# SandroMartens/DBGSOM

Measured on AMD Instinct MI355X. Metric: samples/sec/epoch (BMU+update), higher is better.
Workload: dtype f64; 1 GPU; Synthetic N=1e6 d=784 fp32, M=1024 (32x32); samples_total=1000000, samples_per_gpu=1000000, features=784, prototypes=1024, x_storage=f32, map=frozen (same prototypes every step), bmu_algorithm=filtered, via=HipBackend -> dbgsom_ctx_epoch (one C-ABI call per step)

## Files before the change

dbgsom_amd/_native.py:

```python
from __future__ import annotations

import ctypes
import os
import subprocess

_HERE = os.path.dirname(os.path.abspath(__file__))
CSRC = os.path.join(_HERE, "csrc")
LIB_PATH = os.environ.get("DBGSOM_LIB") or os.path.join(CSRC, "libdbgsom_hip.so")
HEADER = os.path.join(os.path.dirname(_HERE), "include", "dbgsom_hip.h")

F32, F64, BF16 = 0, 1, 2
ALG_AUTO, ALG_EXACT, ALG_FILTERED, ALG_FILTERED_HINT = 0, 1, 2, 3
ALGORITHMS = {"auto": ALG_AUTO, "exact": ALG_EXACT, "filtered": ALG_FILTERED,
              "filtered_hint": ALG_FILTERED_HINT}
EPOCH_FROZEN = 1
ABI_VERSION = 4
ALLREDUCE_FN = ctypes.CFUNCTYPE(ctypes.c_int, ctypes.c_void_p, ctypes.c_void_p, ctypes.c_int64,
                                ctypes.c_void_p)
COLLECTIVE_FN = ctypes.CFUNCTYPE(ctypes.c_int, ctypes.c_void_p, ctypes.c_int, ctypes.c_void_p, ctypes.c_int64,
                                 ctypes.c_void_p)
COLL_ALLREDUCE, COLL_REDUCE_SCATTER, COLL_ALLGATHER = 0, 1, 2
CENTRES_COMPACT, CENTRES_ALIGNED = 0, 1
LAYOUTS = {"compact": CENTRES_COMPACT, "aligned": CENTRES_ALIGNED}
MAX_PROTOTYPES = 16000
SC_COUNTS = ("samples", "iterations", "max_iterations", "drops", "degenerate", "early_stops", "aa_retries",
             "overflow", "max_active", "multi_drops", "g_rows")

_i64, _vp, _ci, _dbl, _sz = (ctypes.c_int64, ctypes.c_void_p, ctypes.c_int, ctypes.c_double,
                             ctypes.c_size_t)

SIGNATURES = {
    "dbgsom_abi_version": (_ci, []),
    "dbgsom_last_error": (ctypes.c_char_p, []),
    "dbgsom_device_count": (_ci, [ctypes.POINTER(_ci)]),
    "dbgsom_row_sqnorms": (_ci, [_vp, _ci, _i64, _i64, _i64, _vp, _vp]),
    "dbgsom_bmu": (_ci, [_vp, _ci, _i64, _i64, _i64, _vp, _vp, _i64, _vp, _ci, _ci, _vp, _vp, _vp]),
    "dbgsom_exp_similarity": (_ci, [_vp, _i64, _dbl, _vp, _vp]),
    "dbgsom_accumulate_workspace_bytes": (_sz, [_i64, _i64, _i64]),
    "dbgsom_accumulate": (_ci, [_vp, _ci, _i64, _i64, _i64, _vp, _vp, _vp, _i64, _vp, _vp, _vp,
                                _sz, _vp]),
    "dbgsom_smooth_workspace_bytes": (_sz, [_i64, _i64]),
    "dbgsom_smooth": (_ci, [_vp, _i64, _i64, _vp, _dbl, _ci, _vp, _vp, _vp, _vp, _sz, _vp]),
    "dbgsom_filter_planes_bytes": (_sz, [_i64, _i64]),
    "dbgsom_filter_prepare": (_ci, [_vp, _ci, _i64, _i64, _i64, _vp, _sz, _vp]),
    "dbgsom_bmu_filtered_workspace_bytes": (_sz, [_i64, _i64, _i64]),
    "dbgsom_bmu_filtered": (_ci, [_vp, _ci, _i64, _i64, _i64, _vp, _vp, _vp, _i64, _vp, _vp, _vp,
                                  _ci, _ci, _ci, _vp, _vp, _vp, _sz, _vp]),
    "dbgsom_bmu_filtered_counts": (_ci, [_vp, _i64, _i64, _i64, _vp, _i64, _vp]),
    "dbgsom_bmu_filtered_counts_async": (_ci, [_vp, _i64, _i64, _i64, _vp, _i64, _vp]),
    "dbgsom_bmu_filtered_refine_counts": (_ci, [_vp, _i64, _i64, _i64, _vp, _vp]),
    "dbgsom_bmu_filtered_gaps": (_ci, [_vp, _i64, _i64, _i64, _vp, _vp]),
    "dbgsom_bmu_filtered_anchored": (_ci, [_vp, _ci, _i64, _i64, _i64, _vp, _vp, _vp, _i64, _vp, _vp, _ci, _vp, _vp,
                                           _ci, _ci, _ci, _vp, _vp, _vp, _sz, _vp]),
    "dbgsom_bmu_filtered_anchor_seeds": (_ci, [_vp, _i64, _i64, _i64, _ci, _vp, _vp, _vp]),
    "dbgsom_filter_timing": (_ci, [_ci]),
    "dbgsom_bmu_filtered_stage_ms": (_ci, [_vp]),
    "dbgsom_sum_workspace_bytes": (_sz, []),
    "dbgsom_sum_f64": (_ci, [_vp, _i64, _vp, _vp, _sz, _vp]),
    "dbgsom_column_sums": (_ci, [_vp, _ci, _i64, _i64, _i64, _vp, _vp, _vp]),
    "dbgsom_topographic_count": (_ci, [_vp, _i64, _vp, _i64, _vp, _vp]),
    "dbgsom_density_terms": (_ci, [_vp, _i64, _dbl, _vp, _vp]),
    "dbgsom_class_histogram": (_ci, [_vp, _vp, _i64, _i64, _i64, _vp, _vp]),
    "dbgsom_ctx_create": (_ci, [_ci, ctypes.POINTER(_vp)]),
    "dbgsom_ctx_destroy": (_ci, [_vp]),
    "dbgsom_ctx_set_option": (_ci, [_vp, ctypes.c_char_p, _i64]),
    "dbgsom_ctx_get_option": (_ci, [_vp, ctypes.c_char_p, ctypes.POINTER(_i64)]),
    "dbgsom_ctx_stream": (_ci, [_vp, ctypes.POINTER(_vp)]),
    "dbgsom_ctx_load": (_ci, [_vp, _vp, _ci, _i64, _i64, _ci]),
    "dbgsom_ctx_load_device": (_ci, [_vp, _vp, _ci, _i64, _i64, _i64]),
    "dbgsom_ctx_read_samples": (_ci, [_vp, _vp, _i64, _vp]),
    "dbgsom_ctx_set_labels": (_ci, [_vp, _vp, _i64]),
    "dbgsom_ctx_set_sample_weight": (_ci, [_vp, _vp, _i64]),
    "dbgsom_ctx_weight_total": (_ci, [_vp, _vp]),
    "dbgsom_ctx_weighted_column_sums": (_ci, [_vp, _vp, _vp]),
    "dbgsom_ctx_class_histogram_weighted": (_ci, [_vp, _vp, _i64, _i64, _vp]),
    "dbgsom_accumulate_weighted_workspace_bytes": (_sz, [_i64, _i64, _i64]),
    "dbgsom_accumulate_weighted": (_ci, [_vp, _ci, _i64, _i64, _i64, _vp, _vp, _vp, _vp, _i64, _vp, _vp, _vp,
                                         _sz, _vp]),
    "dbgsom_weighted_sum_f64": (_ci, [_vp, _vp, _i64, _vp, _vp, _sz, _vp]),
    "dbgsom_topographic_weight": (_ci, [_vp, _vp, _i64, _vp, _i64, _vp, _vp, _sz, _vp]),
    "dbgsom_class_histogram_weighted": (_ci, [_vp, _vp, _vp, _vp, _i64, _i64, _i64, _vp, _vp]),
    "dbgsom_weighted_column_sums_workspace_bytes": (_sz, [_i64]),
    "dbgsom_weighted_column_sums": (_ci, [_vp, _ci, _i64, _i64, _i64, _vp, _vp, _vp, _vp, _sz, _vp]),
    "dbgsom_ctx_set_topology": (_ci, [_vp, _vp, _i64]),
    "dbgsom_ctx_set_allreduce": (_ci, [_vp, _vp, _vp]),
    "dbgsom_ctx_set_collectives": (_ci, [_vp, _vp, _vp, _ci, _ci]),
    "dbgsom_rccl_unique_id": (_ci, [_vp]),
    "dbgsom_rccl_comm_init": (_ci, [_vp, _ci, _ci, ctypes.POINTER(_vp)]),
    "dbgsom_rccl_comm_destroy": (_ci, [_vp]),
    "dbgsom_ctx_set_rccl": (_ci, [_vp, _vp]),
    "dbgsom_ctx_allreduce_host": (_ci, [_vp, _vp, _i64]),
    "dbgsom_ctx_set_weights": (_ci, [_vp, _vp, _i64]),
    "dbgsom_ctx_get_weights": (_ci, [_vp, _ci, _vp, _i64]),
    "dbgsom_ctx_read_weight_rows": (_ci, [_vp, _ci, _vp, _i64, _vp]),
    "dbgsom_ctx_write_weight_rows": (_ci, [_vp, _i64, _i64, _vp]),
    "dbgsom_ctx_bmu": (_ci, [_vp, _vp, _i64, _ci, _ci, _vp, _vp]),
    "dbgsom_ctx_bmu_query": (_ci, [_vp, _vp, _ci, _i64, _i64, _vp, _i64, _ci, _ci, _vp, _vp]),
    "dbgsom_ctx_bmu_query_device": (_ci, [_vp, _vp, _ci, _i64, _i64, _i64, _vp, _i64, _ci, _ci, _vp, _vp]),
    "dbgsom_ctx_sparse_code_device": (_ci, [_vp, _vp, _ci, _i64, _i64, _i64, _vp, _i64, _ci, _vp, _i64, _vp, _vp,
                                            _vp]),
    "dbgsom_ctx_topographic_function_device": (_ci, [_vp, _vp, _ci, _i64, _i64, _i64, _vp, _i64, _ci, _vp, _i64, _vp,
                                                     _vp, _vp]),
    "dbgsom_sparse_code_workspace_bytes": (_sz, [_i64, _i64, _i64, _ci]),
    "dbgsom_sparse_code": (_ci, [_vp, _ci, _i64, _i64, _i64, _vp, _i64, _i64, _ci, _ci, _vp, _i64, _vp, _vp, _vp,
                                 _vp, _sz, _vp]),
    "dbgsom_sparse_code_timing": (_ci, [_ci]),
    "dbgsom_sparse_code_stage_ms": (_ci, [_vp]),
    "dbgsom_csr_check": (_ci, [_vp, _vp, _i64, _i64, _i64]),
    "dbgsom_csr_row_sqnorms": (_ci, [_vp, _vp, _ci, _i64, _vp, _vp]),
    "dbgsom_csr_wt_ld": (_i64, [_i64]),
    "dbgsom_csr_transpose_weights": (_ci, [_vp, _i64, _i64, _i64, _vp, _i64, _vp]),
    "dbgsom_bmu_csr": (_ci, [_vp, _vp, _vp, _ci, _i64, _vp, _vp, _i64, _i64, _vp, _ci, _ci, _vp, _vp, _vp]),
    "dbgsom_csr_densify": (_ci, [_vp, _vp, _vp, _ci, _i64, _i64, _i64, _vp, _vp]),
    "dbgsom_accumulate_csr_workspace_bytes": (_sz, [_i64, _i64, _i64]),
    "dbgsom_accumulate_csr": (_ci, [_vp, _vp, _vp, _ci, _i64, _i64, _vp, _vp, _vp, _vp, _i64, _vp, _vp, _vp, _sz,
                                    _vp]),
    "dbgsom_ctx_load_csr": (_ci, [_vp, _vp, _vp, _vp, _ci, _i64, _i64, _i64]),
    "dbgsom_ctx_bmu_query_csr": (_ci, [_vp, _vp, _vp, _vp, _ci, _i64, _i64, _i64, _vp, _i64, _ci, _ci, _vp, _vp]),
    "dbgsom_ctx_sparse_code": (_ci, [_vp, _vp, _ci, _i64, _i64, _vp, _i64, _ci, _vp, _i64, _vp, _vp, _vp]),
    "dbgsom_bmu_masked_workspace_bytes": (_sz, [_ci, _i64, _i64, _i64]),
    "dbgsom_bmu_masked": (_ci, [_vp, _ci, _i64, _i64, _i64, _vp, _i64, _i64, _ci, _vp, _vp, _vp, _sz, _vp]),
    "dbgsom_fill_missing": (_ci, [_vp, _ci, _i64, _i64, _i64, _vp, _i64, _i64, _vp, _i64, _vp]),
    "dbgsom_ctx_bmu_query_masked": (_ci, [_vp, _vp, _ci, _i64, _i64, _vp, _i64, _ci, _vp, _vp, _vp]),
    "dbgsom_accumulate_masked_workspace_bytes": (_sz, [_i64, _i64, _i64]),
    "dbgsom_accumulate_masked": (_ci, [_vp, _ci, _i64, _i64, _i64, _vp, _vp, _vp, _i64, _vp, _vp, _vp, _sz, _vp]),
    "dbgsom_smooth_masked_workspace_bytes": (_sz, [_i64, _i64]),
    "dbgsom_smooth_masked": (_ci, [_vp, _i64, _i64, _vp, _dbl, _vp, _vp, _vp, _vp, _sz, _vp]),
    "dbgsom_ctx_bmu_masked": (_ci, [_vp, _vp, _i64, _ci, _vp, _vp]),
    "dbgsom_ctx_epoch_masked": (_ci, [_vp, _vp, _i64, _dbl, _dbl, _vp, _vp, _vp, _vp, _vp, _vp]),
    "dbgsom_topofn_workspace_bytes": (_sz, [_i64, _ci]),
    "dbgsom_topofn": (_ci, [_vp, _i64, _vp, _i64, _i64, _vp, _vp, _vp, _vp, _sz, _vp]),
    "dbgsom_topofn_timing": (_ci, [_ci]),
    "dbgsom_topofn_stage_ms": (_ci, [_vp]),
    "dbgsom_ctx_topographic_function": (_ci, [_vp, _vp, _ci, _i64, _i64, _vp, _i64, _ci, _vp, _i64, _vp, _vp,
                                              _vp]),
    "dbgsom_ctx_exp_similarity": (_ci, [_vp, _vp, _i64, _dbl, _vp]),
    "dbgsom_ctx_epoch": (_ci, [_vp, _vp, _i64, _ci, _dbl, _dbl, _ci, _ci, _vp, _vp, _vp, _vp, _vp,
                               _vp]),
    "dbgsom_ctx_update": (_ci, [_vp, _vp, _i64, _vp, _vp, _vp, _dbl, _ci, _vp, _vp, _vp, _vp]),
    "dbgsom_ctx_set_hint": (_ci, [_vp, _vp, _i64]),
    "dbgsom_ctx_read_sums": (_ci, [_vp, _vp, _i64]),
    "dbgsom_ctx_column_sums": (_ci, [_vp, _vp, _vp]),
    "dbgsom_ctx_quantization_error": (_ci, [_vp, _vp, _i64, _ci, _vp]),
    "dbgsom_ctx_topographic_count": (_ci, [_vp, _vp, _i64, _ci, _vp, _vp]),
    "dbgsom_ctx_node_statistics": (_ci, [_vp, _vp, _i64, _ci, _dbl, _vp, _vp]),
    "dbgsom_ctx_class_histogram": (_ci, [_vp, _vp, _i64, _i64, _vp]),
    "dbgsom_ctx_partition": (_ci, [_vp, _vp, _i64, _ci, _vp, _vp]),
    "dbgsom_ctx_subset_create": (_ci, [_vp, _i64, ctypes.POINTER(_vp)]),
    "dbgsom_ctx_epoch_info": (_ci, [_vp, _vp]),
    "dbgsom_ctx_arm_ms": (_ci, [_vp, _vp]),
    "dbgsom_ctx_filter_counts": (_ci, [_vp, _vp, _i64]),
    "dbgsom_ctx_read_anchors": (_ci, [_vp, ctypes.POINTER(_i64), _vp, _vp, _vp, _vp]),
    "dbgsom_ctx_refine_counts": (_ci, [_vp, _vp]),
    "dbgsom_ctx_phase_ms": (_ci, [_vp, _vp]),
}

_lib = None
_hip_rt = None


class DbgsomNativeError(RuntimeError):

    def __init__(self, fn, code, msg):
        super().__init__(f"{fn} failed ({code}): {msg}")
        self.code = code


def build(verbose: bool = False) -> str:
    out = None if verbose else subprocess.DEVNULL
    subprocess.check_call(["make", "-C", CSRC, "-j4", "libdbgsom_hip.so"], stdout=out)
    return LIB_PATH


def _load_hip_runtime():
    candidates = []
    try:
        import importlib.util

        spec = importlib.util.find_spec("torch")
        if spec and spec.origin:
            candidates.append(os.path.join(os.path.dirname(spec.origin), "lib", "libamdhip64.so"))
    except (ImportError, ValueError):
        pass
    rocm = os.environ.get("ROCM_PATH", "/opt/rocm")
    candidates += [os.path.join(rocm, "lib", "libamdhip64.so"), "libamdhip64.so"]
    errors = []
    for path in candidates:
        if os.path.isabs(path) and not os.path.exists(path):
            continue
        try:
            rt = ctypes.CDLL(path, mode=ctypes.RTLD_GLOBAL)
        except OSError as e:
            errors.append(f"{path}: {e}")
            continue
        rccl = os.path.join(os.path.dirname(path), "librccl.so") if os.path.isabs(path) else ""
        if rccl and os.path.exists(rccl):
            os.environ.setdefault("DBGSOM_RCCL_LIB", rccl)
        return rt
    raise RuntimeError("no HIP runtime (libamdhip64.so) could be loaded: " + "; ".join(errors))


def load():
    global _lib, _hip_rt
    if _lib is not None:
        return _lib
    if not os.path.exists(LIB_PATH):
        raise RuntimeError(
            f"{LIB_PATH} is missing: the HIP extension is not built. Run "
            "`python -c 'import __graft_entry__ as g; g.build()'` (or `make -C dbgsom_amd/csrc`). "
            "dbgsom_amd has no CPU fallback.")
    _hip_rt = _load_hip_runtime()
    lib = ctypes.CDLL(LIB_PATH)
    for name, (res, args) in SIGNATURES.items():
        fn = getattr(lib, name)
        fn.restype = res
        fn.argtypes = args
    if lib.dbgsom_abi_version() != ABI_VERSION:
        raise RuntimeError(f"ABI version mismatch: library {lib.dbgsom_abi_version()}, "
                           f"binding {ABI_VERSION} (rebuild: make -C dbgsom_amd/csrc)")
    _lib = lib
    return lib


def check(fn_name: str, rc: int) -> None:
    if rc != 0:
        msg = load().dbgsom_last_error()
        err = DbgsomNativeError(fn_name, rc, msg.decode(errors="replace") if msg else "")
        if rc == -1:
            raise ValueError(str(err))
        raise err


def call(fn_name: str, *args):
    check(fn_name, getattr(load(), fn_name)(*args))
# ... 7 lines not shown
```

dbgsom_amd/backend.py:

```python
from __future__ import annotations

import ctypes
import os
from dataclasses import dataclass
from typing import Optional

import numpy as np

from . import _native


@dataclass
class EpochResult:
    new_weights: np.ndarray
    change_total: float
    errors: np.ndarray
    activations: np.ndarray
    winners: Optional[np.ndarray] = None
    distances: Optional[np.ndarray] = None
    new_weights_dev: object = None
    class_hist: Optional[np.ndarray] = None


def shard_bounds(n: int, rank: int, world: int):
# ... 253 lines not shown
_RCCL_COMMS = {}


class HipBackend(HotPathBackend):

    name = "hip"

    FILTER_MIN_PROTOTYPES = 129
    FILTER_MAX_FEATURES = 43690
    FILTER_MAX_MEAN_CANDIDATES = 320
    FILTER_MIN_QUERY_ROWS = 32768
    SWEEP_COST = {1: 0.35, 2: 1.0, 3: 1.96}
    LIST_COST = 12.5
    PRUNE_PASS_COST = 60.0

    def __init__(self, device: Optional[int] = None, algorithm: str = "auto", _ctx=None):
        self._lib = _native.load()
        if algorithm not in _native.ALGORITHMS:
            raise ValueError("algorithm must be 'auto', 'exact', 'filtered' or 'filtered_hint'")
        self._init_args = (device, algorithm)
        n_dev = _native.device_count()
        if n_dev < 1:
            raise RuntimeError(
                "dbgsom_amd.HipBackend needs a visible AMD GPU (MI355X / gfx950); found "
                f"hipGetDeviceCount()={n_dev}. There is no CPU fallback in the product path.")
        if device is None:
            device = int(os.environ.get("LOCAL_RANK", "0")) % n_dev
        self.device_index = int(device)
        self._ctx = ctypes.c_void_p()
        if _ctx is not None:
            self._ctx = _ctx
        else:
            _native.call("dbgsom_ctx_create", self.device_index, ctypes.byref(self._ctx))
        self._set("algorithm", _native.ALGORITHMS[algorithm])
        self._loaded = _ctx is not None
        self._borrowed = None
        self._hop_key = None
        self._cb = None
        self._cb_error = None
        self._last_M = 0
        self._x_traffic = {k: 0 for k in self._X_TRAFFIC}
        self.filter_log = []
        self.phase_log = None
        if _ctx is not None:
            self._N, self._d = self._get("n_samples"), self._get("features")
            self._x_np_dtype = {_native.F32: np.dtype(np.float32), _native.F64: np.dtype(np.float64),
                                _native.BF16: "bf16"}[self._get("storage")]
        self._install_collective()

    def _set(self, name, value):
        _native.call("dbgsom_ctx_set_option", self._ctx, name.encode(), int(value))

    def _get(self, name) -> int:
        v = ctypes.c_int64(0)
        _native.call("dbgsom_ctx_get_option", self._ctx, name.encode(), ctypes.byref(v))
        return int(v.value)

    def _call(self, fn, *args):
        self._cb_error = None
        try:
            _native.call(fn, *args)
        except _native.DbgsomNativeError:
            if self._cb_error is not None:
                raise self._cb_error
            raise

    algorithm = property(lambda self: {v: k for k, v in _native.ALGORITHMS.items()}[self._get("algorithm")],
                         lambda self, a: self._set("algorithm", _native.ALGORITHMS[a]))
    sweep_planes = property(lambda self: self._get("sweep_planes"),
                            lambda self, v: self._set("sweep_planes", v))
    seed_stride = property(lambda self: self._get("seed_stride"),
                           lambda self, v: self._set("seed_stride", v))
    refine = property(lambda self: self._get("refine"), lambda self, v: self._set("refine", int(v)))
    refined = property(lambda self: bool(self._get("refined")))
    defer = property(lambda self: bool(self._get("defer")), lambda self, v: self._set("defer", int(bool(v))))
    shard_smooth = property(lambda self: self._get("shard_smooth"), lambda self, v: self._set("shard_smooth", int(v)))
    shard_epochs = property(lambda self: self._get("shard_epochs"))
    defer_epochs = property(lambda self: self._get("defer_epochs"))
    csr_densify_below = property(lambda self: self._get("csr_densify_below"),
                                 lambda self, v: self._set("csr_densify_below", int(v)))
    resident_csr = property(lambda self: bool(self._get("resident_csr")))
    planes_cached = property(lambda self: bool(self._get("planes_cached")))
    anchor_seeds = property(lambda self: self._get("anchor_seeds"), lambda self, v: self._set("anchor_seeds", int(v)))
    anchor_builds = property(lambda self: self._get("anchor_builds"))
    anchor_searches = property(lambda self: self._get("anchor_searches"))
    anchor_state = property(lambda self: self._get("anchor_state"))
    padded_features = property(lambda self: self._get("padded_features"))

    @property
    def n_samples(self):
        return self._get("n_samples")

    def _require_loaded(self):
        if not self._loaded:
            raise RuntimeError("HipBackend: call load(X) first")

    def _install_collective(self):
        rank, world = dist_info()
        force = os.environ.get("DBGSOM_FORCE_COLLECTIVE") == "1" and _group_is_up()
        if world == 1 and not force:
            _native.call("dbgsom_ctx_set_collectives", self._ctx, None, None, 0, 1)
            self._cb = None
            return
        import torch
        import torch.distributed as td

        dev = torch.device("cuda", self.device_index)
        on_device = td.get_backend() == "nccl"
        if on_device and os.environ.get("DBGSOM_COLLECTIVE", "rccl") != "callback":
            key = (self.device_index, world, rank)
            comm = _RCCL_COMMS.get(key, "untried")
            if comm == "untried":
                uid, err = ctypes.create_string_buffer(128), None
                if rank == 0:
                    try:
                        _native.call("dbgsom_rccl_unique_id", uid)
                    except Exception as e:
                        err = e
                box = [uid.raw if err is None else None]
                td.broadcast_object_list(box, src=0)
                comm = ctypes.c_void_p()
                if box[0] is not None:
                    try:
                        uid = ctypes.create_string_buffer(box[0], 128)
                        self._get("n_samples")
                        _native.call("dbgsom_rccl_comm_init", uid, world, rank, ctypes.byref(comm))
                    except Exception as e:
                        err, comm = e, ctypes.c_void_p()
                else:
                    err = err or RuntimeError("rank 0 could not make an RCCL id")
                ok = torch.tensor([1 if (err is None and comm.value) else 0], device=dev, dtype=torch.int32)
                td.all_reduce(ok, op=td.ReduceOp.MIN)
                if int(ok.item()) == 1:
                    _RCCL_COMMS[key] = comm
                else:
                    import warnings
                    warnings.warn(f"dbgsom_amd: RCCL inside the library is unavailable ({err}); "
                                  "collectives go through torch.distributed")
                    _RCCL_COMMS[key] = comm = None
            if comm is not None:
                _native.call("dbgsom_ctx_set_rccl", self._ctx, comm)
                self._cb = None
                return
        cache = {}

        def collective(_user, op, ptr, count, stream):
            try:
                ext = cache.get(("stream", stream))
                if ext is None:
                    ext = cache[("stream", stream)] = torch.cuda.ExternalStream(stream, device=dev)
                total = count if op == _native.COLL_ALLREDUCE else count * world
                with torch.cuda.stream(ext):
                    t = cache.get((ptr, total))
                    if t is None:
                        if len(cache) > 16:
                            cache.clear()
                            cache[("stream", stream)] = ext
                        t = cache[(ptr, total)] = torch.as_tensor(_DeviceArray(ptr, total), device=dev)
                    mine = t[rank * count:(rank + 1) * count] if op != _native.COLL_ALLREDUCE else None
                    if on_device:
                        if op == _native.COLL_ALLREDUCE:
                            td.all_reduce(t, op=td.ReduceOp.SUM)
                        elif op == _native.COLL_REDUCE_SCATTER:
                            td.reduce_scatter_tensor(mine, t, op=td.ReduceOp.SUM)
                        else:
                            td.all_gather_into_tensor(t, mine.clone())
# ... 375 lines not shown
                   None if Wn is None else Wn.ctypes.data, chg.ctypes.data, E.ctypes.data, a.ctypes.data,
                   None if win is None else win.ctypes.data, None if dist is None else dist.ctypes.data)
        self._last_M = M
        res = EpochResult(Wn, float(chg[0]), E, a, win, dist, RESIDENT if keep_on_device else None)
        if n_classes > 0:
            res.class_hist = self.class_histogram(None, n_classes, M)
        self._log_epoch()
        return res

    def epoch_masked(self, W, hop, sigma, gamma, want_assignments=False, n_classes=0):
        self._require_loaded()
        if W is RESIDENT:
            raise ValueError("no prototypes stay resident between masked epochs")
        keep, p, M, _ = self._w_arg(W, d=self._d)
        self._topology(hop, M)
        Wn, chg, E, a = np.empty((M, self._d)), np.empty(1), np.empty(M), np.empty(M)
        want = want_assignments or n_classes > 0
        win = np.empty(self._N, dtype=np.int64) if want else None
        dist = np.empty(self._N) if want else None
        self._call("dbgsom_ctx_epoch_masked", self._ctx, p, M, float(gamma), float(sigma), Wn.ctypes.data,
                   chg.ctypes.data, E.ctypes.data, a.ctypes.data, None if win is None else win.ctypes.data,
                   None if dist is None else dist.ctypes.data)
        self._last_M = M
        res = EpochResult(Wn, float(chg[0]), E, a, win if want_assignments else None, dist if want_assignments else None)
        if n_classes > 0:
            res.class_hist = self.class_histogram(win, n_classes, M)
        return res

    def epoch_info(self):
        info = (ctypes.c_double * 8)()
        _native.call("dbgsom_ctx_epoch_info", self._ctx, info)
        return [float(v) for v in info]

    def arm_ms(self):
        ms = (ctypes.c_double * 12)()
        _native.call("dbgsom_ctx_arm_ms", self._ctx, ms)
        return {(i // 4, i % 4): float(v) for i, v in enumerate(ms) if v == v}

    def _log_epoch(self):
        info = self.epoch_info()
        if info[0]:
            self.filter_log.append(("filtered", float(info[1]), int(info[2])))
        elif self.algorithm != "exact":
            self.filter_log.append(("exact", None))
        del self.filter_log[:-64]
        if self.phase_log is not None:
            ms = (ctypes.c_double * 8)()
            _native.call("dbgsom_ctx_phase_ms", self._ctx, ms)
            self.phase_log.append([float(v) for v in ms])

    def update(self, W, hop, sigma, sample_weights, winners, distances, layout="compact"):
        self._require_loaded()
        keep, p, M, _ = self._w_arg(W)
        self._topology(hop, M)
        idx = np.ascontiguousarray(winners, dtype=np.int64)
        kw = np.ascontiguousarray(sample_weights, dtype=np.float64)
        dist = np.ascontiguousarray(distances, dtype=np.float64)
        if not (idx.size == kw.size == dist.size == self._N):
            raise ValueError("one winner / weight / distance per resident sample")
        Wn, chg, E, a = np.empty((M, self._d)), np.empty(1), np.empty(M), np.empty(M)
        self._call("dbgsom_ctx_update", self._ctx, p, M, idx.ctypes.data, kw.ctypes.data,
                   dist.ctypes.data, float(sigma), _native.LAYOUTS[layout], Wn.ctypes.data,
                   chg.ctypes.data, E.ctypes.data, a.ctypes.data)
        self._last_M = M
        return Wn, float(chg[0]), E, a

    def set_hint(self, winners, M):
        idx = np.ascontiguousarray(winners, dtype=np.int64)
        if idx.size != self._N:
            raise ValueError("one seed per resident sample")
        self._call("dbgsom_ctx_set_hint", self._ctx, idx.ctypes.data, int(M))

    def read_sums(self, M):
        out = np.empty(M * (self._d + 3))
        self._call("dbgsom_ctx_read_sums", self._ctx, out.ctypes.data, int(M))
        return out

    def filter_counts(self):
        nb = (self._N + 127) // 128
        out = np.empty(nb, dtype=np.uint32)
        self._call("dbgsom_ctx_filter_counts", self._ctx, out.ctypes.data, nb)
        return out

    def read_anchors(self, aseed=False):
        n = ctypes.c_int64(0)
        self._call("dbgsom_ctx_read_anchors", self._ctx, ctypes.byref(n), None, None, None, None)
        out = {"anchors": np.empty((n.value, self.padded_features)), "anchor_of": np.empty(self._N, dtype=np.int32),
               "order": np.empty(self._N, dtype=np.int32)}
        if aseed:
            out["aseed"] = np.empty(n.value, dtype=np.int32)
        self._call("dbgsom_ctx_read_anchors", self._ctx, None, out["anchors"].ctypes.data, out["anchor_of"].ctypes.data,
                   out["order"].ctypes.data, out["aseed"].ctypes.data if aseed else None)
        return out

    def refine_counts(self):
        out = np.zeros(4, dtype=np.uint64)
        self._call("dbgsom_ctx_refine_counts", self._ctx, out.ctypes.data)
        return [int(v) for v in out]

    def traffic(self):
        keys = ("w_upload_calls", "w_upload_bytes", "w_download_calls", "w_download_bytes",
                "w_row_writes", "w_row_reads")
        return {k: self._get(k) for k in keys}

    _X_TRAFFIC = ("x_upload_bytes", "x_upload_calls", "x_download_bytes")

    def sample_traffic(self):
        return {k: self._x_traffic[k] + (self._get(k) if self._ctx else 0) for k in self._X_TRAFFIC}

    def plane_cost(self, p, mean, M):
        return self.arm_cost(p, mean, M, self._N, self.padded_features)

    @classmethod
    def arm_cost(cls, p, mean, M, N, dp):
        if p == 0:
            launches = 25.0 / (2.8 * (float(max(N, 1)) * dp) / (1.0e6 * 784.0))
            return (cls.PRUNE_PASS_COST + cls.SWEEP_COST[1] * M * 9.0 * M / max(N, 1) + launches
                    + cls.LIST_COST * mean)
        return cls.SWEEP_COST[p] * M + cls.LIST_COST * mean

    def column_moments(self):
        self._require_loaded()
        if isinstance(self._x_np_dtype, str) or self.resident_csr:
            return None
        s1 = np.empty(self._d, dtype=self._x_np_dtype)
        self._call("dbgsom_ctx_column_sums", self._ctx, None, s1.ctypes.data)
        mean = np.ascontiguousarray(np.true_divide(s1, self._N))
        s2 = np.empty_like(s1)
        self._call("dbgsom_ctx_column_sums", self._ctx, mean.ctypes.data, s2.ctypes.data)
        return s1, s2, self._N

    _weighted = False
    _incomplete = False

    def set_sample_weight(self, w):
        self._require_loaded()
        super().set_sample_weight(w)
        if w is None:
            self._call("dbgsom_ctx_set_sample_weight", self._ctx, None, 0)
        else:
            self._call("dbgsom_ctx_set_sample_weight", self._ctx, self._sw.ctypes.data, self._sw.size)
        self._weighted = w is not None

    def weight_total(self) -> float:
        out = np.empty(1)
        self._call("dbgsom_ctx_weight_total", self._ctx, out.ctypes.data)
        return float(out[0])

    def weighted_column_moments(self, total):
        self._require_loaded()
        s1 = np.empty(self._d)
        self._call("dbgsom_ctx_weighted_column_sums", self._ctx, None, s1.ctypes.data)
        mean = np.ascontiguousarray(s1 / total)
        s2 = np.empty(self._d)
        self._call("dbgsom_ctx_weighted_column_sums", self._ctx, mean.ctypes.data, s2.ctypes.data)
        return s1, s2

    def quantization_error(self, W) -> float:
        self._require_loaded()
        if self._incomplete:
            return super().quantization_error(W)
        keep, p, M, rf = self._w_arg(W)
        out = np.empty(2)
        self._call("dbgsom_ctx_quantization_error", self._ctx, p, M, rf, out.ctypes.data)
        return float(out[0] / out[1])

    def topographic_error_count(self, W, coords) -> int:
        self._require_loaded()
        if self._incomplete:
            return super().topographic_error_count(W, coords)
        keep, p, M, rf = self._w_arg(W)
        xy = np.ascontiguousarray(coords, dtype=np.int32)
        if xy.shape != (M, 2):
            raise ValueError("coords must be (M, 2)")
        out = np.empty(1)
        self._call("dbgsom_ctx_topographic_count", self._ctx, p, M, rf, xy.ctypes.data, out.ctypes.data)
        return float(out[0]) if self._weighted else int(round(out[0]))

    def node_statistics(self, W, sigma):
        self._require_loaded()
        if self._incomplete:
            return super().node_statistics(W, sigma)
        keep, p, M, rf = self._w_arg(W)
        hits, dens = np.empty(M), np.empty(M)
        self._call("dbgsom_ctx_node_statistics", self._ctx, p, M, rf, float(sigma), hits.ctypes.data,
                   dens.ctypes.data)
        return hits, dens

    def set_labels(self, y):
        super().set_labels(y)
        if y is None:
            self._call("dbgsom_ctx_set_labels", self._ctx, None, 0)
        else:
            self._call("dbgsom_ctx_set_labels", self._ctx, self._y.ctypes.data, self._y.size)

    def class_histogram(self, winners, n_classes, M):
        if self._incomplete:
            return super().class_histogram(winners, n_classes, M)
        idx = None if winners is None else np.ascontiguousarray(winners, dtype=np.int64)
        if self._weighted:
            hist = np.empty((M, n_classes), dtype=np.float64)
            self._call("dbgsom_ctx_class_histogram_weighted", self._ctx, None if idx is None else idx.ctypes.data,
                       int(n_classes), int(M), hist.ctypes.data)
            return hist
        hist = np.empty((M, n_classes), dtype=np.int64)
        self._call("dbgsom_ctx_class_histogram", self._ctx, None if idx is None else idx.ctypes.data,
                   int(n_classes), int(M), hist.ctypes.data)
        return hist

    def partition(self, W, want_winners=False):
        self._require_loaded()
        keep, p, M, rf = self._w_arg(W)
        counts = np.empty(M, dtype=np.int64)
        win = np.empty(self._N, dtype=np.int64) if want_winners else None
        self._call("dbgsom_ctx_partition", self._ctx, p, M, rf, counts.ctypes.data,
                   None if win is None else win.ctypes.data)
        return counts, win

    def subset(self, neuron):
        child = ctypes.c_void_p()
        self._call("dbgsom_ctx_subset_create", self._ctx, int(neuron), ctypes.byref(child))
        sub = HipBackend(self.device_index, self.algorithm, _ctx=child)
        sub._weighted = self._weighted
        return sub

    _SETTABLE = ("algorithm", "sweep_planes", "seed_stride", "timing", "graph", "refine", "defer",
                 "filter_min_query_rows", "max_mean_candidates", "shard_smooth", "csr_densify_below", "anchor_seeds")

    def release(self):
        if self._ctx:
            opts = {k: self._get(k) for k in self._SETTABLE}
            for k in self._X_TRAFFIC:
                self._x_traffic[k] += self._get(k)
            _native.call("dbgsom_ctx_destroy", self._ctx)
            self._ctx = ctypes.c_void_p()
            _native.call("dbgsom_ctx_create", self.device_index, ctypes.byref(self._ctx))
            for k, v in opts.items():
                self._set(k, v)
            self._install_collective()
        self._loaded = False
        self._borrowed = None
        self._hop_key = None
        self._weighted = False
        self._incomplete = False
        self._sw = None

    def __del__(self):
        try:
            if getattr(self, "_ctx", None):
                self._lib.dbgsom_ctx_destroy(self._ctx)
                self._ctx = None
        except Exception:
            pass
```

dbgsom_amd/csrc/common.h:

```cpp
#pragma once
#include <hip/hip_runtime.h>
#include <stdint.h>
#include <stdio.h>

#include "../../include/dbgsom_hip.h"

namespace dbgsom {

void set_error(const char *fmt, ...);

#define DBGSOM_HIP_CHECK(expr)                                                           \
    do {                                                                                 \
        hipError_t _e = (expr);                                                          \
        if (_e != hipSuccess) {                                                          \
            ::dbgsom::set_error("%s failed: %s (%s:%d)", #expr, hipGetErrorString(_e),   \
                                __FILE__, __LINE__);                                     \
            return DBGSOM_EHIP;                                                          \
        }                                                                                \
    } while (0)

#define DBGSOM_REQUIRE(cond, msg)                                   \
    do {                                                            \
        if (!(cond)) {                                              \
            ::dbgsom::set_error("%s: %s", __func__, msg);           \
// ... 126 lines not shown
struct StageTimer {
    bool enabled = false, valid = false;
    hipEvent_t ev[6] = {};
    bool created = false;
    void mark(int k, hipStream_t s) {
        if (!enabled) return;
        if (!created) { for (auto &e : ev) (void)hipEventCreate(&e); created = true; }
        (void)hipEventRecord(ev[k], s);
    }
    void destroy() {
        if (created) for (auto &e : ev) (void)hipEventDestroy(e);
        created = false; valid = false;
    }
};

struct SideStream {
    hipStream_t stream = nullptr, stream2 = nullptr;
    hipEvent_t forked = nullptr, joined = nullptr, joined2 = nullptr, mid = nullptr;
    hipEvent_t gap_fork = nullptr, gap_done = nullptr;
    int state = 0;
    int device = -1;
    bool ready() {
        int dev = -1;
        if (hipGetDevice(&dev) != hipSuccess) return false;
        if (state == 0) {
            device = dev;
            int prio_low = 0, prio_high = 0;
            (void)hipDeviceGetStreamPriorityRange(&prio_low, &prio_high);
            state = (hipStreamCreateWithPriority(&stream, hipStreamNonBlocking, prio_low) == hipSuccess &&
                     hipStreamCreateWithPriority(&stream2, hipStreamNonBlocking, prio_low) == hipSuccess &&
                     hipEventCreateWithFlags(&forked, hipEventDisableTiming) == hipSuccess &&
                     hipEventCreateWithFlags(&joined, hipEventDisableTiming) == hipSuccess &&
                     hipEventCreateWithFlags(&joined2, hipEventDisableTiming) == hipSuccess &&
                     hipEventCreateWithFlags(&mid, hipEventDisableTiming) == hipSuccess &&
                     hipEventCreateWithFlags(&gap_fork, hipEventDisableTiming) == hipSuccess &&
                     hipEventCreateWithFlags(&gap_done, hipEventDisableTiming) == hipSuccess) ? 1 : -1;
        }
        return state == 1 && dev == device;
    }
    void destroy() {
        if (state == 1) {
            (void)hipStreamDestroy(stream); (void)hipStreamDestroy(stream2);
            for (hipEvent_t e : {forked, joined, joined2, mid, gap_fork, gap_done}) (void)hipEventDestroy(e);
        }
        state = 0;
    }
};

struct FilterAux {
    StageTimer timer;
    SideStream side;
    void destroy() { timer.destroy(); side.destroy(); }
};
int filter_stage_ms(FilterAux &aux, double *ms5);

struct FilteredCall {
    const void *X = nullptr;
    int x_dtype = 0;
    int64_t N = 0, d = 0, ldx = 0;
    const double *xx = nullptr;
    const void *xplanes = nullptr;
    const double *W = nullptr;
    int64_t M = 0;
    const double *ww = nullptr;
    const int64_t *prev_idx = nullptr;
    const int32_t *order = nullptr;
    int seed_stride = 0, sweep_planes = 0, round_f32 = 0;
    int k = 1;
    int64_t *idx = nullptr;
    double *dist = nullptr;
    void *ws = nullptr;
    size_t ws_bytes = 0;
    hipStream_t stream = nullptr;
    const double *hint_dist = nullptr, *hint_shift = nullptr;
    int refine_rows = 0;
    bool defer_dist = false;
    const void *X_store = nullptr;
    int store_dtype = -1;
    int64_t ld_store = 0;
    double guard_mean = 0.0;
    const double *anchors = nullptr;
    const int32_t *anchor_of = nullptr;
    int n_anchors = 0;
    int32_t *seeds_out = nullptr, *order_out = nullptr;
    FilterAux *aux = nullptr;
};
constexpr int DBGSOM_LISTS_LONG = 1000;
int launch_bmu_filtered(const FilteredCall &call);
size_t smooth_workspace_bytes(int64_t M, int64_t d);
int launch_smooth(const double *sums, int64_t M, int64_t d, const float *hop, double sigma,
                  int layout, const double *W_old, double *W_new, double *change_total, void *ws,
                  size_t ws_bytes, hipStream_t s);
int64_t smooth_block_cols(int64_t d, int nranks);
int64_t smooth_block_elems(int64_t M, int64_t d, int nranks);
int launch_pack_blocks(const double *sums, int64_t M, int64_t d, int nranks, double *out, hipStream_t s);
int launch_smooth_block(const double *S_b, const double *K, const double *a, int64_t M, int64_t cb, int64_t d_full,
                        const float *hop, double sigma, int layout, double *Wb, void *ws, size_t ws_bytes,
                        hipStream_t s);
int launch_rowchange_blocks(const double *blocks, int64_t M, int64_t d, int64_t cb, const double *W_old, double *W_new,
                            double *change_total, void *ws, hipStream_t s);

}
```

dbgsom_amd/csrc/engine.hip:

```cpp
#include <dlfcn.h>
#include <math.h>
#include <stdlib.h>
#include <string.h>

#include <chrono>
#include <new>
#include <vector>

#include "anchor_chain.h"
#include "common.h"
#include "search_policy.h"

namespace dbgsom {

struct DevBuf {
    void *p = nullptr;
    size_t cap = 0;
    bool tight = false;
    int reserve(size_t bytes) {
        if (bytes <= cap) return DBGSOM_OK;
        if (p) { (void)hipFree(p); p = nullptr; cap = 0; }
        const size_t want = tight ? align_up(bytes) : align_up(bytes + bytes / 8, 1 << 20);
        hipError_t e = hipMalloc(&p, want);
        if (e != hipSuccess) {
            p = nullptr;
            (void)hipGetLastError();
            set_error("hipMalloc(%zu) failed: %s", want, hipGetErrorString(e));
            return DBGSOM_ENOMEM;
        }
        cap = want;
        return DBGSOM_OK;
    }
    int reserve_zeroed(size_t bytes, hipStream_t s) {
        if (bytes <= cap) return DBGSOM_OK;
        const int rc = reserve(bytes);
        if (rc != DBGSOM_OK) return rc;
        hipError_t e = hipMemsetAsync(p, 0, cap, s);
        if (e != hipSuccess) { set_error("hipMemsetAsync failed: %s", hipGetErrorString(e)); return DBGSOM_EHIP; }
        return DBGSOM_OK;
    }
    int reserve_keep(size_t bytes, size_t keep, hipStream_t s) {
        if (bytes <= cap) return DBGSOM_OK;
        void *old = p;
        const size_t old_cap = cap;
        p = nullptr;
        cap = 0;
        const int rc = reserve(bytes * 2);
        if (rc != DBGSOM_OK) { p = old; cap = old_cap; return rc; }
        if (old && keep) {
            hipError_t e = hipMemcpyAsync(p, old, keep, hipMemcpyDeviceToDevice, s);
            if (e == hipSuccess) e = hipStreamSynchronize(s);
            if (e != hipSuccess) { set_error("device copy failed: %s", hipGetErrorString(e)); (void)hipFree(old); return DBGSOM_EHIP; }
        }
        if (old) (void)hipFree(old);
        return DBGSOM_OK;
    }
    void release() { if (p) (void)hipFree(p); p = nullptr; cap = 0; }
    template <typename T> T *as() const { return reinterpret_cast<T *>(p); }
};

struct PinBuf {
    void *p = nullptr;
    size_t cap = 0;
    int reserve(size_t bytes) {
        if (bytes <= cap) return DBGSOM_OK;
        if (p) { (void)hipHostFree(p); p = nullptr; cap = 0; }
        const size_t want = align_up(bytes * 2, 4096);
        hipError_t e = hipHostMalloc(&p, want, hipHostMallocMapped);
        if (e == hipSuccess) e = hipHostGetDevicePointer(&dev, p, 0);
        if (e != hipSuccess) { if (p) (void)hipHostFree(p); p = nullptr; dev = nullptr; (void)hipGetLastError(); set_error("hipHostMalloc(%zu) failed: %s", want, hipGetErrorString(e)); return DBGSOM_ENOMEM; }
        cap = want;
        return DBGSOM_OK;
    }
    void *dev = nullptr;
    void release() { if (p) (void)hipHostFree(p); p = nullptr; dev = nullptr; cap = 0; }
    template <typename T> T *as() const { return reinterpret_cast<T *>(p); }
};

__global__ void round_bf16_kernel(float *__restrict__ x, uint16_t *__restrict__ out, int64_t n) {
    for (int64_t i = (int64_t)blockIdx.x * blockDim.x + threadIdx.x; i < n; i += (int64_t)gridDim.x * blockDim.x) {
        const uint32_t u = __float_as_uint(x[i]);
        uint16_t b;
        if ((u & 0x7fffffffu) > 0x7f800000u) b = 0x7fc0;
        else b = (uint16_t)((u + 0x7fffu + ((u >> 16) & 1u)) >> 16);
        out[i] = b;
        x[i] = __uint_as_float(((uint32_t)b) << 16);
    }
}
__global__ void widen_bf16_kernel(const uint16_t *__restrict__ in, float *__restrict__ out, int64_t n) {
    for (int64_t i = (int64_t)blockIdx.x * blockDim.x + threadIdx.x; i < n; i += (int64_t)gridDim.x * blockDim.x)
        out[i] = __uint_as_float(((uint32_t)in[i]) << 16);
}
__global__ void f64_to_f32_kernel(const double *__restrict__ in, float *__restrict__ out, int64_t n) {
// ... 18 lines not shown
    }
    __threadfence_system();
}
__global__ __launch_bounds__(64) void row_shift_kernel(const double *__restrict__ A, const double *__restrict__ B,
                                                       int64_t ld, int64_t d, int64_t rows, int64_t M,
                                                       double *__restrict__ shift) {
    const int64_t p = blockIdx.x;
    if (p >= M) return;
    if (p >= rows) { if (threadIdx.x == 0) shift[p] = INFINITY; return; }
    double acc = 0.0;
    if (A != B)
        for (int64_t k = threadIdx.x; k < d; k += 64) {
            const double t = A[p * ld + k] - B[p * ld + k];
            acc = fma(t, t, acc);
        }
    for (int off = 32; off > 0; off >>= 1) acc += __shfl_xor(acc, off, 64);
    if (threadIdx.x == 0) shift[p] = sqrt(acc) * (1.0 + 1e-9);
}
__global__ void status_to_f64_kernel(const int32_t *__restrict__ status, double *__restrict__ out) {
    out[0] = status[0] ? 1.0 : 0.0;
}
template <typename T>
__global__ void gather_rows_kernel(const T *__restrict__ src, int64_t ld, const int32_t *__restrict__ ids,
                                   int64_t first, int64_t n, int64_t cols, T *__restrict__ dst) {
    const int64_t r = blockIdx.x;
    if (r >= n) return;
    const T *s = src + (int64_t)ids[first + r] * ld;
    T *d = dst + r * cols;
    for (int64_t c = threadIdx.x; c < cols; c += blockDim.x) d[c] = s[c];
}
__global__ void gather_f64_kernel(const double *__restrict__ src, const int32_t *__restrict__ ids, int64_t first,
                                  int64_t n, double *__restrict__ dst) {
    for (int64_t i = (int64_t)blockIdx.x * blockDim.x + threadIdx.x; i < n; i += (int64_t)gridDim.x * blockDim.x)
        dst[i] = src[ids[first + i]];
}
__global__ void gather_i32_kernel(const int32_t *__restrict__ src, const int32_t *__restrict__ ids, int64_t first,
                                  int64_t n, int32_t *__restrict__ dst) {
    for (int64_t i = (int64_t)blockIdx.x * blockDim.x + threadIdx.x; i < n; i += (int64_t)gridDim.x * blockDim.x)
        dst[i] = src[ids[first + i]];
}
template <typename T>
__global__ void rows_to_f64_kernel(const T *__restrict__ src, int64_t ld, const int64_t *__restrict__ ids, int64_t n,
                                   int64_t cols, double *__restrict__ dst) {
    const int64_t r = blockIdx.x;
    if (r >= n) return;
    const T *s = src + ids[r] * ld;
    for (int64_t c = threadIdx.x; c < cols; c += blockDim.x) dst[r * cols + c] = widen(s[c]);
}
__global__ void iota_i32_kernel(int32_t *__restrict__ a, int32_t *__restrict__ b, int64_t n) {
    for (int64_t i = (int64_t)blockIdx.x * blockDim.x + threadIdx.x; i < n; i += (int64_t)gridDim.x * blockDim.x)
        a[i] = b[i] = (int32_t)i;
}
__global__ void seg_counts_kernel(const uint32_t *__restrict__ seg_start, int64_t M, int64_t N, int64_t *__restrict__ counts) {
    for (int64_t j = (int64_t)blockIdx.x * blockDim.x + threadIdx.x; j < M; j += (int64_t)gridDim.x * blockDim.x)
        counts[j] = (int64_t)((j + 1 < M ? seg_start[j + 1] : (uint32_t)N) - seg_start[j]);
}

static unsigned grid1d(int64_t n, int block = 256) {
    const int64_t nb = (n + block - 1) / block;
    return (unsigned)(nb < 1 ? 1 : (nb > 8192 ? 8192 : nb));
}

}

using namespace dbgsom;

extern "C" {
const unsigned long long *dbgsom_filter_count_sum_ptr(const void *workspace_dev, int64_t N, int64_t d, int64_t M);
size_t dbgsom_filter_planes_bytes(int64_t rows, int64_t d);
size_t dbgsom_bmu_filtered_workspace_bytes(int64_t N, int64_t d, int64_t M);
}

namespace {

struct Samples {
    int dtype = -1;
    int64_t N = 0, d = 0, dp = 0;
    const void *X = nullptr;
    const void *Xb = nullptr;
    int bdtype = -1;
    DevBuf own, x32, xx, planes;
    bool planes_ready = false;
    DevBuf anchors, anchor_of, anchor_order;
    int64_t n_anchors = 0;
    int anchor_state = 0;
    void drop_anchors(int state) {
        anchors.release(); anchor_of.release(); anchor_order.release();
        n_anchors = 0; anchor_state = state;
    }
    void drop_planes() { planes_ready = false; drop_anchors(0); }
    bool csr = false;
    int64_t nnz = 0;
    DevBuf indptr, indices, data;
    CsrView view() const { return CsrView{indptr.as<int64_t>(), indices.as<int32_t>(), data.p}; }
    void release() {
        own.release(); x32.release(); xx.release(); planes.release(); indptr.release(); indices.release(); data.release();
        drop_planes(); csr = false; nnz = 0; dtype = -1; N = 0; X = Xb = nullptr;
    }
};

}

struct dbgsom_ctx {
    int device = 0;
    hipStream_t stream = nullptr;
    int timing = 0;
    int use_graph = 0;
    int defer = 0;
    bool last_deferred = false;
    int64_t defer_epochs = 0;
    int last_round_f32 = 0;
    bool last_refined = false;
    bool last_k2_filtered = false;
    int64_t filter_min_query_rows = 32768;
    int64_t sc_chunk_rows = 32768;
    int64_t sc_cap = 0;
    DevBuf sc_ws, sc_x, sc_w, sc_p, sc_code, sc_proba, sc_cnt;
    int64_t masked_chunk_rows = 32768;
    DevBuf mk_ws, mk_x, mk_w, mk_idx, mk_dist;
    bool incomplete = false;
    DevBuf mf_nobs, mf_x64, mf_wt, mf_w, mf_wn, mf_idx, mf_dist, mf_kw, mf_sums, mf_acc_ws, mf_sm_ws, mf_scal;
    Samples xs, xq;
    DevBuf y;
    bool has_labels = false;
    DevBuf sw, wh_order, wh_ws;
    bool has_weights = false;
    int64_t topoM = 0;
    DevBuf hop, hop_stage;
    DevBuf Wb[2];
    int cur = 0;
    int64_t M = 0;
    int64_t otherM = 0;
    DevBuf ww, idx[2], dist, kw, sums, acc_ws, sm_ws, filt_ws, scal, qidx, qdist, red, hist, stage_dev;
    DevBuf wt;
    int64_t csr_densify_below = 1024;
    int icur = 0;
    bool hint_valid = false;
    int64_t hintM = 0;
    bool last_idx_valid = false;
    int64_t sumsM = 0;
    DevBuf part_order, part_ws, part_counts;
    int64_t partM = 0;
    bool part_valid = false;
    SearchPolicy policy;
    bool dist_bound_valid = false;
    int distW_buf = 0;
    int64_t distW_M = 0;
    DevBuf shiftb;
    bool last_filtered = false;
    int64_t last_filter_M = 0, last_filter_N = 0, last_filter_d = 0;
    const void *last_filter_ws = nullptr;
    PinBuf tail, counts;
    dbgsom_allreduce_fn allreduce = nullptr;
    void *allreduce_user = nullptr;
    void *rccl_comm = nullptr;
    bool rccl_owned = false;
    dbgsom_collective_fn coll = nullptr;
    void *coll_user = nullptr;
    int coll_rank = 0, coll_nranks = 1;
    int shard_smooth = 2;
    bool sums_sharded = false;
    int64_t shard_epochs = 0;
    DevBuf shard_send, shard_gather;
    int64_t w_up_calls = 0, w_up_bytes = 0, w_down_calls = 0, w_down_bytes = 0, w_row_writes = 0, w_row_reads = 0;
    int64_t x_up_bytes = 0, x_up_calls = 0, x_down_bytes = 0;
    void x_up(size_t bytes) { x_up_bytes += (int64_t)bytes; ++x_up_calls; }
    void x_down(size_t bytes) { x_down_bytes += (int64_t)bytes; }
    hipEvent_t ev[4] = {};
    bool ev_created = false, ev_valid = false;
    double filter_ms[5] = {0, 0, 0, 0, 0};
    bool filter_ms_valid = false;
    FilterAux faux;
    int anchor_seeds = 1;
    int64_t anchor_builds = 0, anchor_searches = 0;
    bool anchors_built_now = false;
    bool last_anchor_seeded = false;
    double prepass_mean = NAN;
    int64_t prepass_M = 0;
};

namespace {

#define CTX_CHECK(c)                                                                 \
    do {                                                                             \
        if (!(c)) { set_error("%s: null context", __func__); return DBGSOM_EINVAL; } \
        DBGSOM_HIP_CHECK(hipSetDevice((c)->device));                                 \
    } while (0)
#define TRY(expr) do { int _rc = (expr); if (_rc != DBGSOM_OK) return _rc; } while (0)

inline int64_t pad16(int64_t d) { return (d + 15) / 16 * 16; }

int sync(dbgsom_ctx *c) {
    DBGSOM_HIP_CHECK(hipStreamSynchronize(c->stream));
    return DBGSOM_OK;
}

int upload_padded(dbgsom_ctx *c, void *dst, const void *src, int64_t rows, int64_t d, int64_t dp, size_t es) {
    if (rows == 0) return DBGSOM_OK;
    if (d == dp) {
        DBGSOM_HIP_CHECK(hipMemcpyAsync(dst, src, (size_t)rows * d * es, hipMemcpyHostToDevice, c->stream));
    } else {
        DBGSOM_HIP_CHECK(hipMemsetAsync(dst, 0, (size_t)rows * dp * es, c->stream));
        DBGSOM_HIP_CHECK(hipMemcpy2DAsync(dst, (size_t)dp * es, src, (size_t)d * es, (size_t)d * es, (size_t)rows,
                                          hipMemcpyHostToDevice, c->stream));
    }
    return DBGSOM_OK;
}

int download_unpadded(dbgsom_ctx *c, void *dst, const void *src, int64_t rows, int64_t d, int64_t dp, size_t es) {
    if (rows == 0) return DBGSOM_OK;
    if (d == dp)
        DBGSOM_HIP_CHECK(hipMemcpyAsync(dst, src, (size_t)rows * d * es, hipMemcpyDeviceToHost, c->stream));
    else
        DBGSOM_HIP_CHECK(hipMemcpy2DAsync(dst, (size_t)d * es, src, (size_t)dp * es, (size_t)d * es, (size_t)rows,
                                          hipMemcpyDeviceToHost, c->stream));
    return DBGSOM_OK;
}

int finish_samples(dbgsom_ctx *c, Samples &s, bool x32_is_widened) {
    if (s.dtype == DBGSOM_BF16) {
        if (!x32_is_widened) {
            TRY(s.x32.reserve((size_t)s.N * s.dp * 4));
            hipLaunchKernelGGL(widen_bf16_kernel, dim3(grid1d(s.N * s.dp)), dim3(256), 0, c->stream,
                               (const uint16_t *)s.X, s.x32.as<float>(), s.N * s.dp);
            TRY(launch_status("widen_bf16_kernel"));
        }
        s.Xb = s.x32.p;
        s.bdtype = DBGSOM_F32;
    } else {
        s.Xb = s.X;
        s.bdtype = s.dtype;
    }
    TRY(s.xx.reserve((size_t)s.N * 8));
    TRY(launch_row_sqnorms(s.Xb, s.bdtype, s.N, s.dp, s.dp, s.xx.as<double>(), c->stream));
    s.drop_planes();
    return DBGSOM_OK;
}

int place_host_samples(dbgsom_ctx *c, Samples &s, const void *X_host, int x_dtype, int64_t N, int64_t d, int storage) {
    DBGSOM_REQUIRE(valid_dtype(x_dtype) && valid_dtype(storage), "dtype must be DBGSOM_F32/F64/BF16");
    DBGSOM_REQUIRE(X_host && N >= 1 && d >= 1 && N < 0x7fffffff, "bad samples");
    DBGSOM_REQUIRE(storage == x_dtype || (storage == DBGSOM_BF16 && x_dtype == DBGSOM_F32),
                   "storage must be the input dtype, or DBGSOM_BF16 for float32 input");
    const int64_t dp = pad16(d);
    s.N = N; s.d = d; s.dp = dp; s.dtype = storage;
    s.csr = false; s.nnz = 0;
    bool widened = false;
    if (storage == DBGSOM_BF16 && x_dtype == DBGSOM_F32) {
        TRY(s.x32.reserve((size_t)N * dp * 4));
        TRY(s.own.reserve((size_t)N * dp * 2));
        TRY(upload_padded(c, s.x32.p, X_host, N, d, dp, 4));
        hipLaunchKernelGGL(round_bf16_kernel, dim3(grid1d(N * dp)), dim3(256), 0, c->stream, s.x32.as<float>(),
                           s.own.as<uint16_t>(), N * dp);
        TRY(launch_status("round_bf16_kernel"));
        widened = true;
    } else {
        const size_t es = dtype_size(x_dtype);
        TRY(s.own.reserve((size_t)N * dp * es));
        TRY(upload_padded(c, s.own.p, X_host, N, d, dp, es));
    }
    s.X = s.own.p;
    c->x_up((size_t)N * d * dtype_size(x_dtype));
    return finish_samples(c, s, widened);
}

bool device_rows_conform(const void *X_dev, int64_t d, int64_t ldx) {
    return ldx == pad16(d) && d == ldx && is_aligned(X_dev, 16);
}

int place_device_samples(dbgsom_ctx *c, Samples &s, const void *X_dev, int x_dtype, int64_t N, int64_t d, int64_t ldx) {
    DBGSOM_REQUIRE(valid_dtype(x_dtype), "x_dtype must be DBGSOM_F32/F64/BF16");
    DBGSOM_REQUIRE(X_dev && N >= 1 && d >= 1 && ldx >= d && N < 0x7fffffff, "bad samples");
    const size_t es = dtype_size(x_dtype);
    const int64_t dp = pad16(d);
    s.dtype = -1;
    s.N = N; s.d = d; s.dp = dp;
    s.csr = false; s.nnz = 0;
    s.indptr.release(); s.indices.release(); s.data.release();
    if (device_rows_conform(X_dev, d, ldx)) {
        s.own.release();
        s.X = X_dev;
    } else {
        TRY(s.own.reserve((size_t)N * dp * es));
        if (d != dp) DBGSOM_HIP_CHECK(hipMemsetAsync(s.own.p, 0, (size_t)N * dp * es, c->stream));
        DBGSOM_HIP_CHECK(hipMemcpy2DAsync(s.own.p, (size_t)dp * es, X_dev, (size_t)ldx * es, (size_t)d * es, (size_t)N,
                                          hipMemcpyDeviceToDevice, c->stream));
        s.X = s.own.p;
    }
    s.dtype = x_dtype;
    return finish_samples(c, s, false);
}

struct QueryRows {
    const void *p;
    bool on_device;
    int64_t ldx;
};

int place_query_rows(dbgsom_ctx *c, Samples &s, const QueryRows &q, int x_dtype, int64_t Nq, int64_t d) {
    if (q.on_device) return place_device_samples(c, s, q.p, x_dtype, Nq, d, q.ldx);
    return place_host_samples(c, s, q.p, x_dtype, Nq, d, x_dtype);
}

void drop_query_rows(Samples &s, const QueryRows &q, int64_t held_bytes) {
    if (q.on_device && s.X != s.own.p) { s.X = s.Xb = nullptr; s.dtype = -1; s.drop_planes(); }
    if (held_bytes > ((int64_t)256 << 20)) s.release();
}

int ensure_planes(dbgsom_ctx *c, Samples &s) {
    if (s.planes_ready) return DBGSOM_OK;
    const size_t nbytes = dbgsom_filter_planes_bytes(s.N, s.dp);
    TRY(s.planes.reserve(nbytes));
    TRY(dbgsom_filter_prepare(s.Xb, s.bdtype, s.N, s.dp, s.dp, s.planes.p, s.planes.cap, c->stream));
    s.planes_ready = true;
    return DBGSOM_OK;
}

int gather_anchor_rows(dbgsom_ctx *c, Samples &s, const std::vector<int64_t> &rows, double *anchors) {
    const int64_t A = (int64_t)rows.size(), dp = s.dp;
    TRY(c->stage_dev.reserve((size_t)A * 8));
    int64_t *ids = c->stage_dev.as<int64_t>();
    DBGSOM_HIP_CHECK(hipMemcpyAsync(ids, rows.data(), (size_t)A * 8, hipMemcpyHostToDevice, c->stream));
    DBGSOM_HIP_CHECK(hipStreamSynchronize(c->stream));
    if (s.dtype == DBGSOM_F32)
        hipLaunchKernelGGL(rows_to_f64_kernel<float>, dim3((unsigned)A), dim3(256), 0, c->stream, (const float *)s.X, dp, ids, A, dp, anchors);
    else if (s.dtype == DBGSOM_F64)
        hipLaunchKernelGGL(rows_to_f64_kernel<double>, dim3((unsigned)A), dim3(256), 0, c->stream, (const double *)s.X, dp, ids, A, dp, anchors);
    else
        hipLaunchKernelGGL(rows_to_f64_kernel<bf16_t>, dim3((unsigned)A), dim3(256), 0, c->stream, (const bf16_t *)s.X, dp, ids, A, dp, anchors);
    TRY(launch_status("rows_to_f64_kernel"));
    return DBGSOM_OK;
}

int ensure_anchors(dbgsom_ctx *c, Samples &s) {
    if (s.anchor_state != 0) return DBGSOM_OK;
    TRY(ensure_planes(c, s));
    const int64_t A = s.N < 256 ? s.N : 256, dp = s.dp;
    TRY(s.anchors.reserve((size_t)A * dp * 8 + (size_t)A * 8));
    TRY(s.anchor_of.reserve((size_t)s.N * 4));
    TRY(s.anchor_order.reserve((size_t)s.N * 4));
    std::vector<int64_t> rows = anchor_rows(s.N, A);
    double *anchors = s.anchors.as<double>(), *anorm = anchors + (size_t)A * dp;
    TRY(gather_anchor_rows(c, s, rows, anchors));
    if (A < s.N && A > 2) {
        std::vector<double> host((size_t)A * dp);
        DBGSOM_HIP_CHECK(hipMemcpyAsync(host.data(), anchors, (size_t)A * dp * 8, hipMemcpyDeviceToHost, c->stream));
        DBGSOM_HIP_CHECK(hipStreamSynchronize(c->stream));
        chain_anchors(host, A, dp, rows);
        TRY(gather_anchor_rows(c, s, rows, anchors));
    }
    if (A == s.N) {
        hipLaunchKernelGGL(iota_i32_kernel, dim3(grid1d(s.N)), dim3(256), 0, c->stream, s.anchor_of.as<int32_t>(),
                           s.anchor_order.as<int32_t>(), s.N);
        TRY(launch_status("iota_i32_kernel"));
    } else {
        TRY(launch_row_sqnorms(anchors, DBGSOM_F64, A, dp, dp, anorm, c->stream));
        TRY(c->filt_ws.reserve_zeroed(dbgsom_bmu_filtered_workspace_bytes(s.N, dp, A), c->stream));
        FilteredCall call;
        call.aux = &c->faux;
        call.X = s.Xb; call.x_dtype = s.bdtype; call.N = s.N; call.d = dp; call.ldx = dp;
        call.xx = s.xx.as<double>(); call.xplanes = s.planes.p; call.W = anchors; call.M = A; call.ww = anorm;
        call.seed_stride = DBGSOM_SEED_FULL; call.sweep_planes = 1;
        call.seeds_out = s.anchor_of.as<int32_t>(); call.order_out = s.anchor_order.as<int32_t>();
        call.ws = c->filt_ws.p; call.ws_bytes = c->filt_ws.cap; call.stream = c->stream;
        TRY(launch_bmu_filtered(call));
    }
    s.n_anchors = A;
    s.anchor_state = 1;
    ++c->anchor_builds;
    c->anchors_built_now = true;
    return DBGSOM_OK;
}

bool filter_shape_ok(const Samples &s, int64_t M) { return SearchPolicy::shape_ok(M, s.N, s.dp); }

bool filter_applies(const dbgsom_ctx *c, int64_t M) {
    if (c->xs.csr) return false;
    return c->policy.filter_allowed() && filter_shape_ok(c->xs, M);
}

bool hint_applies(const dbgsom_ctx *c, int64_t M) { return c->policy.takes_hint() && c->hint_valid && c->hintM <= M; }

int stage_weights(dbgsom_ctx *c, const double *W_host, int64_t M, int64_t d, int64_t dp) {
    DBGSOM_REQUIRE(M >= 1 && M <= 0x7fffff00, "bad prototype count");
    if (W_host) {
        TRY(c->Wb[c->cur].reserve((size_t)M * dp * 8));
        TRY(upload_padded(c, c->Wb[c->cur].p, W_host, M, d, dp, 8));
        if (c->distW_buf == c->cur) c->dist_bound_valid = false;
        c->M = M;
        ++c->w_up_calls; c->w_up_bytes += M * d * 8;
    } else if (c->M != M) {
        set_error("no resident prototypes of %lld rows (resident: %lld); pass W_host or call dbgsom_ctx_set_weights",
                  (long long)M, (long long)c->M);
        return DBGSOM_ESTATE;
    }
    TRY(c->ww.reserve((size_t)M * 8));
    return launch_row_sqnorms(c->Wb[c->cur].p, DBGSOM_F64, M, dp, dp, c->ww.as<double>(), c->stream);
}

int run_filtered(dbgsom_ctx *c, Samples &s, DevBuf &ws, const double *W, int64_t M, int round_f32,
                 const int64_t *prev_idx, const int32_t *order, int64_t *idx, double *dist, bool may_probe = false,
                 bool allow_defer = false) {
    TRY(ensure_planes(c, s));
    TRY(ws.reserve_zeroed(dbgsom_bmu_filtered_workspace_bytes(s.N, s.dp, M), c->stream));
    const bool bound_usable = c->dist_bound_valid && dist == c->dist.as<double>() && c->Wb[c->distW_buf].p;
    const SearchPolicy::Plan plan = c->policy.plan(M, s.N, s.dp, prev_idx != nullptr, may_probe, bound_usable);
    FilteredCall call;
    call.aux = &c->faux;
    if (plan.hint_bound) {
        TRY(c->shiftb.reserve((size_t)M * 8));
        const int64_t rows = c->distW_M < M ? c->distW_M : M;
        hipLaunchKernelGGL(row_shift_kernel, dim3((unsigned)M), dim3(64), 0, c->stream, W,
                           c->Wb[c->distW_buf].as<double>(), s.dp, s.dp, rows, M, c->shiftb.as<double>());
        TRY(launch_status("row_shift_kernel"));
        call.hint_dist = c->dist.as<double>();
        call.hint_shift = c->shiftb.as<double>();
    }
    call.X = s.Xb; call.x_dtype = s.bdtype; call.N = s.N; call.d = s.dp; call.ldx = s.dp;
    call.xx = s.xx.as<double>(); call.xplanes = s.planes.p; call.W = W; call.M = M; call.ww = c->ww.as<double>();
    call.prev_idx = prev_idx; call.order = order; call.seed_stride = plan.seed_stride; call.sweep_planes = plan.sweep_planes;
    c->last_anchor_seeded = false;
    const bool has_ref = c->prepass_mean == c->prepass_mean && SearchPolicy::near_size(M, c->prepass_M);
    if (!prev_idx && &s == &c->xs && c->anchor_seeds && s.anchor_state != 2 && has_ref && plan.planes == 0 &&
        !plan.seed_full && (plan.seed_stride & DBGSOM_PRUNE)) {
        TRY(ensure_anchors(c, s));
        ++c->anchor_searches;
        call.anchors = s.anchors.as<double>(); call.n_anchors = (int)s.n_anchors;
        call.anchor_of = s.anchor_of.as<int32_t>(); call.order = s.anchor_order.as<int32_t>();
        c->last_anchor_seeded = true;
    }
    call.round_f32 = round_f32; call.idx = idx; call.dist = dist; call.ws = ws.p; call.ws_bytes = ws.cap;
    call.stream = c->stream;
    call.refine_rows = plan.refine_rows;
    c->last_refined = plan.refine;
    call.defer_dist = plan.refine && allow_defer && c->defer && M < 0xffff &&
                      accumulate_can_fill_distances(s.dtype, s.dp);
    c->last_deferred = call.defer_dist;
    c->last_round_f32 = round_f32;
    if (s.dtype == DBGSOM_BF16) { call.X_store = s.X; call.store_dtype = DBGSOM_BF16; call.ld_store = s.dp; }
    call.guard_mean = plan.guard_mean;
    const int rc_f = launch_bmu_filtered(call);
    c->last_filter_M = M; c->last_filter_N = s.N; c->last_filter_d = s.dp; c->last_filter_ws = ws.p;
    if (rc_f == DBGSOM_LISTS_LONG) {
        c->policy.on_guarded();
        c->last_refined = false;
        c->last_deferred = false;
        return launch_bmu(s.Xb, s.bdtype, s.N, s.dp, s.dp, s.xx.as<double>(), W, M, c->ww.as<double>(), 1, round_f32, idx,
                          dist, c->stream);
    }
    TRY(rc_f);
    return DBGSOM_OK;
}

struct RcclApi {
    int (*get_unique_id)(void *id) = nullptr;
    int (*comm_init_rank)(void **comm, int nranks,  ...) = nullptr;
    int (*all_reduce)(const void *, void *, size_t, int, int, void *, hipStream_t) = nullptr;
    int (*reduce_scatter)(const void *, void *, size_t, int, int, void *, hipStream_t) = nullptr;
    int (*all_gather)(const void *, void *, size_t, int, void *, hipStream_t) = nullptr;
    int (*comm_count)(void *, int *) = nullptr;
    int (*comm_user_rank)(void *, int *) = nullptr;
    int (*comm_destroy)(void *) = nullptr;
    const char *(*error_string)(int) = nullptr;
    bool tried = false, ok = false;
};
struct NcclUniqueId { char internal[128]; };
typedef int (*nccl_comm_init_rank_fn)(void **comm, int nranks, NcclUniqueId id, int rank);
RcclApi g_rccl;
nccl_comm_init_rank_fn g_rccl_init = nullptr;

int rccl_load() {
    if (g_rccl.tried) {
        if (!g_rccl.ok) { set_error("librccl could not be loaded (see the first failure)"); return DBGSOM_ESTATE; }
        return DBGSOM_OK;
    }
    g_rccl.tried = true;
    void *h = nullptr;
    const bool in_process = dlsym(RTLD_DEFAULT, "ncclAllReduce") != nullptr;
    if (in_process) h = RTLD_DEFAULT;
    const char *env = getenv("DBGSOM_RCCL_LIB");
    const char *names[] = {env, "librccl.so", "librccl.so.1", "/opt/rocm/lib/librccl.so"};
    for (const char *n : names) {
        if (in_process || h) break;
        if (n && *n) h = dlopen(n, RTLD_NOW | RTLD_GLOBAL);
    }
    if (!h && !in_process) { set_error("librccl not found (set DBGSOM_RCCL_LIB): %s", dlerror()); return DBGSOM_ESTATE; }
    g_rccl.get_unique_id = (int (*)(void *))dlsym(h, "ncclGetUniqueId");
    g_rccl_init = (nccl_comm_init_rank_fn)dlsym(h, "ncclCommInitRank");
    g_rccl.all_reduce = (int (*)(const void *, void *, size_t, int, int, void *, hipStream_t))dlsym(h, "ncclAllReduce");
    g_rccl.comm_destroy = (int (*)(void *))dlsym(h, "ncclCommDestroy");
    g_rccl.reduce_scatter = (int (*)(const void *, void *, size_t, int, int, void *, hipStream_t))dlsym(h, "ncclReduceScatter");
    g_rccl.all_gather = (int (*)(const void *, void *, size_t, int, void *, hipStream_t))dlsym(h, "ncclAllGather");
    g_rccl.comm_count = (int (*)(void *, int *))dlsym(h, "ncclCommCount");
    g_rccl.comm_user_rank = (int (*)(void *, int *))dlsym(h, "ncclCommUserRank");
    g_rccl.error_string = (const char *(*)(int))dlsym(h, "ncclGetErrorString");
    g_rccl.ok = g_rccl.get_unique_id && g_rccl_init && g_rccl.all_reduce && g_rccl.comm_destroy;
    if (!g_rccl.ok) { set_error("librccl lacks ncclGetUniqueId / ncclCommInitRank / ncclAllReduce / ncclCommDestroy"); return DBGSOM_ESTATE; }
    return DBGSOM_OK;
}
const char *rccl_err(int rc) { return g_rccl.error_string ? g_rccl.error_string(rc) : "?"; }
void drop_rccl(dbgsom_ctx *c) {
    if (c->rccl_comm && c->rccl_owned && g_rccl.ok) {
        if (c->stream) (void)hipStreamSynchronize(c->stream);
        (void)g_rccl.comm_destroy(c->rccl_comm);
    }
    if (c->rccl_comm) { c->coll_rank = 0; c->coll_nranks = 1; }
    c->rccl_comm = nullptr;
    c->rccl_owned = false;
}

int run_allreduce(dbgsom_ctx *c, double *buf, int64_t count) {
// ... 385 lines not shown
    hipError_t err = hipStreamCreateWithPriority(&c->stream, hipStreamNonBlocking, prio_high);
    if (err != hipSuccess) { (void)hipGetLastError(); err = hipStreamCreateWithFlags(&c->stream, hipStreamNonBlocking); }
    if (err != hipSuccess) {
        set_error("hipStreamCreate failed: %s", hipGetErrorString(err));
        delete c;
        return DBGSOM_EHIP;
    }
    *out = c;
    return DBGSOM_OK;
}

#define CTX_DEVBUFS(c)                                                                                             \
    {&(c)->y, &(c)->hop, &(c)->hop_stage, &(c)->Wb[0], &(c)->Wb[1], &(c)->ww, &(c)->idx[0], &(c)->idx[1], &(c)->dist,  \
     &(c)->kw, &(c)->sums, &(c)->acc_ws, &(c)->sm_ws, &(c)->filt_ws, &(c)->scal, &(c)->qidx, &(c)->qdist, &(c)->red,  \
     &(c)->hist, &(c)->stage_dev, &(c)->part_order, &(c)->part_ws, &(c)->part_counts, &(c)->shiftb, &(c)->shard_send,    \
     &(c)->shard_gather, &(c)->sw, &(c)->wh_order, &(c)->wh_ws, &(c)->sc_ws, &(c)->sc_x, &(c)->sc_w, &(c)->sc_p, &(c)->sc_code, &(c)->sc_proba, &(c)->sc_cnt, &(c)->wt,  \
     &(c)->mk_ws, &(c)->mk_x, &(c)->mk_w, &(c)->mk_idx, &(c)->mk_dist, &(c)->mf_nobs, &(c)->mf_x64, &(c)->mf_wt, &(c)->mf_w,   \
     &(c)->mf_wn, &(c)->mf_idx, &(c)->mf_dist, &(c)->mf_kw, &(c)->mf_sums, &(c)->mf_acc_ws, &(c)->mf_sm_ws, &(c)->mf_scal}

int dbgsom_ctx_destroy(dbgsom_ctx *c) {
    if (!c) return DBGSOM_OK;
    (void)hipSetDevice(c->device);
    if (c->stream) (void)hipStreamSynchronize(c->stream);
    drop_rccl(c);
    c->faux.destroy();
    c->xs.release(); c->xq.release();
    DevBuf *bufs[] = CTX_DEVBUFS(c);
    for (DevBuf *b : bufs) b->release();
    c->tail.release(); c->counts.release();
    if (c->ev_created) for (auto &e : c->ev) (void)hipEventDestroy(e);
    if (c->stream) (void)hipStreamDestroy(c->stream);
    delete c;
    return DBGSOM_OK;
}

int dbgsom_ctx_set_option(dbgsom_ctx *c, const char *name, int64_t v) {
    CTX_CHECK(c);
    DBGSOM_REQUIRE(name, "null option name");
    if (!strcmp(name, "algorithm")) {
        DBGSOM_REQUIRE(v >= DBGSOM_ALG_AUTO && v <= DBGSOM_ALG_FILTERED_HINT, "algorithm must be a DBGSOM_ALG_* value");
        c->policy.algorithm = (int)v;
    } else if (!strcmp(name, "sweep_planes")) {
        DBGSOM_REQUIRE(v >= 0 && v <= 4, "sweep_planes must be 0 .. 4 (4 = no sweep: triangle pruning)");
        c->policy.sweep_planes = (int)v;
    } else if (!strcmp(name, "seed_stride")) {
        DBGSOM_REQUIRE(v >= 0 && v <= 64, "seed_stride outside [0, 64]");
        c->policy.seed_stride = (int)v;
    } else if (!strcmp(name, "timing")) {
        c->timing = v != 0;
        c->ev_valid = false;
        c->faux.timer.enabled = c->timing != 0;
        c->faux.timer.valid = false;
    } else if (!strcmp(name, "graph")) {
        c->use_graph = v != 0;
    } else if (!strcmp(name, "defer")) {
        c->defer = v != 0;
    } else if (!strcmp(name, "shard_smooth")) {
        DBGSOM_REQUIRE(v >= 0 && v <= 2, "shard_smooth must be 0 (never), 1 (whenever the collective can) or 2 (large maps)");
        c->shard_smooth = (int)v;
    } else if (!strcmp(name, "refine")) {
        DBGSOM_REQUIRE(v >= 0 && v <= 2, "refine must be 0 (off), 1 (on) or 2 (by measurement)");
        c->policy.set_refine((int)v);
    } else if (!strcmp(name, "filter_min_query_rows")) {
        DBGSOM_REQUIRE(v >= 0, "filter_min_query_rows must be >= 0");
        c->filter_min_query_rows = v;
    } else if (!strcmp(name, "sc_chunk_rows")) {
        DBGSOM_REQUIRE(v >= 1 && v <= ((int64_t)1 << 22), "sc_chunk_rows must be in [1, 2^22]");
        c->sc_chunk_rows = v;
    } else if (!strcmp(name, "masked_chunk_rows")) {
        DBGSOM_REQUIRE(v >= 1 && v <= ((int64_t)1 << 22), "masked_chunk_rows must be in [1, 2^22]");
        c->masked_chunk_rows = v;
    } else if (!strcmp(name, "sc_cap")) {
        DBGSOM_REQUIRE(v >= 0 && v <= 64, "sc_cap must be in [0, 64] (0 = the library's cap)");
        c->sc_cap = v;
    } else if (!strcmp(name, "max_mean_candidates")) {
        DBGSOM_REQUIRE(v >= 1, "max_mean_candidates must be >= 1");
        c->policy.max_mean_candidates = v;
    } else if (!strcmp(name, "csr_densify_below")) {
        DBGSOM_REQUIRE(v >= 0, "csr_densify_below must be >= 0 (0 = CSR input always stays CSR)");
        c->csr_densify_below = v;
    } else if (!strcmp(name, "anchor_seeds")) {
        DBGSOM_REQUIRE(v == 0 || v == 1, "anchor_seeds must be 0 or 1");
        c->anchor_seeds = (int)v;
    } else if (!strcmp(name, "incomplete")) {
        DBGSOM_REQUIRE(v == 0 || v == 1, "incomplete must be 0 or 1");
        c->incomplete = false;
        if (v == 0) { c->mf_nobs.release(); c->mf_x64.release(); return DBGSOM_OK; }
        TRY(loaded(c, __func__));
        Samples &s = c->xs;
        DBGSOM_REQUIRE(!s.csr && (s.dtype == DBGSOM_F32 || s.dtype == DBGSOM_F64),
                       "only dense float32 / float64 residents can be marked incomplete");
        DBGSOM_REQUIRE(!c->has_weights && c->coll_nranks == 1 && !c->allreduce,
                       "incomplete rows take neither sample weights nor more than one rank");
        TRY(c->mf_nobs.reserve((size_t)s.N * 4));
        if (s.dtype == DBGSOM_F32) TRY(c->mf_x64.reserve((size_t)s.N * s.d * 8));
        TRY(launch_masked_prepare(s.X, s.dtype, s.N, s.d, s.dp, c->mf_nobs.as<int32_t>(), c->mf_x64.as<double>(), c->stream));
        TRY(sync(c));
        c->incomplete = true;
    } else {
        set_error("dbgsom_ctx_set_option: unknown option '%s'", name);
        return DBGSOM_EINVAL;
    }
    return DBGSOM_OK;
}

int dbgsom_ctx_get_option(dbgsom_ctx *c, const char *name, int64_t *v) {
    CTX_CHECK(c);
    DBGSOM_REQUIRE(name && v, "null pointer");
    if (!strcmp(name, "algorithm")) *v = c->policy.algorithm;
    else if (!strcmp(name, "sweep_planes")) *v = c->policy.sweep_planes;
    else if (!strcmp(name, "seed_stride")) *v = c->policy.seed_stride;
    else if (!strcmp(name, "timing")) *v = c->timing;
    else if (!strcmp(name, "graph")) *v = c->use_graph;
    else if (!strcmp(name, "refine")) *v = c->policy.refine;
    else if (!strcmp(name, "refined")) *v = c->last_refined ? 1 : 0;
    else if (!strcmp(name, "defer")) *v = c->defer;
    else if (!strcmp(name, "shard_smooth")) *v = c->shard_smooth;
    else if (!strcmp(name, "shard_epochs")) *v = c->shard_epochs;
    else if (!strcmp(name, "defer_epochs")) *v = c->defer_epochs;
    else if (!strcmp(name, "guarded_calls")) *v = c->policy.guarded_calls;
    else if (!strcmp(name, "collective_rank")) *v = c->coll_rank;
    else if (!strcmp(name, "collective_ranks")) *v = c->coll_nranks;
    else if (!strcmp(name, "k2_filtered")) *v = c->last_k2_filtered ? 1 : 0;
    else if (!strcmp(name, "filter_min_query_rows")) *v = c->filter_min_query_rows;
    else if (!strcmp(name, "max_mean_candidates")) *v = c->policy.max_mean_candidates;
    else if (!strcmp(name, "sc_chunk_rows")) *v = c->sc_chunk_rows;
    else if (!strcmp(name, "sc_cap")) *v = c->sc_cap;
    else if (!strcmp(name, "masked_chunk_rows")) *v = c->masked_chunk_rows;
    else if (!strcmp(name, "csr_densify_below")) *v = c->csr_densify_below;
    else if (!strcmp(name, "resident_csr")) *v = (c->xs.dtype >= 0 && c->xs.csr) ? 1 : 0;
    else if (!strcmp(name, "resident_nnz")) *v = (c->xs.dtype >= 0 && c->xs.csr) ? c->xs.nnz : 0;
    else if (!strcmp(name, "n_samples")) *v = c->xs.dtype < 0 ? 0 : c->xs.N;
    else if (!strcmp(name, "features")) *v = c->xs.dtype < 0 ? 0 : c->xs.d;
    else if (!strcmp(name, "padded_features")) *v = c->xs.dtype < 0 ? 0 : c->xs.dp;
    else if (!strcmp(name, "storage")) *v = c->xs.dtype;
    else if (!strcmp(name, "prototypes")) *v = c->M;
    else if (!strcmp(name, "planes_cached")) *v = c->xs.planes_ready ? 1 : 0;
    else if (!strcmp(name, "anchor_seeds")) *v = c->anchor_seeds;
    else if (!strcmp(name, "incomplete")) *v = c->incomplete ? 1 : 0;
    else if (!strcmp(name, "anchor_builds")) *v = c->anchor_builds;
    else if (!strcmp(name, "anchor_searches")) *v = c->anchor_searches;
    else if (!strcmp(name, "anchor_state")) *v = c->xs.dtype < 0 ? 0 : c->xs.anchor_state;
    else if (!strcmp(name, "planes_used")) *v = c->policy.planes_used;
    else if (!strcmp(name, "planes_next")) *v = c->policy.planes_for_call();
    else if (!strcmp(name, "hint_valid")) *v = c->hint_valid ? 1 : 0;
    else if (!strcmp(name, "filter_backoff")) *v = c->policy.filter_backoff;
    else if (!strcmp(name, "plane_hold")) *v = c->policy.plane_hold;
    else if (!strcmp(name, "seed_mode")) *v = c->policy.seed_mode;
    else if (!strcmp(name, "prune_retry")) *v = c->policy.prune_retry ? 1 : 0;
    else if (!strcmp(name, "w_upload_calls")) *v = c->w_up_calls;
    else if (!strcmp(name, "w_upload_bytes")) *v = c->w_up_bytes;
    else if (!strcmp(name, "w_download_calls")) *v = c->w_down_calls;
    else if (!strcmp(name, "w_download_bytes")) *v = c->w_down_bytes;
    else if (!strcmp(name, "w_row_writes")) *v = c->w_row_writes;
    else if (!strcmp(name, "w_row_reads")) *v = c->w_row_reads;
    else if (!strcmp(name, "x_upload_bytes")) *v = c->x_up_bytes;
    else if (!strcmp(name, "x_upload_calls")) *v = c->x_up_calls;
    else if (!strcmp(name, "x_download_bytes")) *v = c->x_down_bytes;
    else if (!strcmp(name, "device_bytes")) {
        size_t tot = 0;
        for (const Samples *q : {&c->xs, &c->xq})
            tot += q->own.cap + q->x32.cap + q->xx.cap + q->planes.cap + q->indptr.cap + q->indices.cap + q->data.cap +
                   q->anchors.cap + q->anchor_of.cap + q->anchor_order.cap;
        DevBuf *bufs[] = CTX_DEVBUFS(c);
        for (DevBuf *b : bufs) tot += b->cap;
        *v = (int64_t)tot;
    } else {
        set_error("dbgsom_ctx_get_option: unknown option '%s'", name);
        return DBGSOM_EINVAL;
    }
    return DBGSOM_OK;
}

int dbgsom_ctx_stream(dbgsom_ctx *c, void **stream) {
    CTX_CHECK(c);
    DBGSOM_REQUIRE(stream, "null pointer");
    *stream = (void *)c->stream;
    return DBGSOM_OK;
}

static void set_tight(dbgsom_ctx *c, bool tight) {
    DevBuf *bufs[] = CTX_DEVBUFS(c);
    for (DevBuf *b : bufs) b->tight = tight;
    for (Samples *q : {&c->xs, &c->xq})
        for (DevBuf *b : {&q->own, &q->x32, &q->xx, &q->planes, &q->indptr, &q->indices, &q->data, &q->anchors, &q->anchor_of,
                          &q->anchor_order})
            b->tight = tight;
}

static void reset_training_state(dbgsom_ctx *c) {
    c->hint_valid = c->last_idx_valid = c->part_valid = false;
    c->has_labels = false;
    c->has_weights = false;
    c->incomplete = false;
    c->policy.reset();
    c->prepass_mean = NAN;
    c->last_anchor_seeded = false;
    c->dist_bound_valid = false;
    c->last_filtered = false;
    c->sumsM = 0;
    c->M = c->otherM = 0;
}

int dbgsom_ctx_load(dbgsom_ctx *c, const void *X_host, int x_dtype, int64_t N, int64_t d, int storage) {
    CTX_CHECK(c);
    reset_training_state(c);
    set_tight(c, false);
    c->xs.dtype = -1;
    c->xs.indptr.release(); c->xs.indices.release(); c->xs.data.release();
    const int rc = place_host_samples(c, c->xs, X_host, x_dtype, N, d, storage);
    if (rc != DBGSOM_OK) { (void)hipStreamSynchronize(c->stream); c->xs.dtype = -1; return rc; }
    return sync(c);
}

int dbgsom_ctx_load_csr(dbgsom_ctx *c, const int64_t *indptr_host, const int32_t *indices_host, const void *data_host,
                        int x_dtype, int64_t N, int64_t d, int64_t nnz) {
    CTX_CHECK(c);
    reset_training_state(c);
    c->xs.dtype = -1;
    set_tight(c, d >= c->csr_densify_below);
    int rc = place_host_csr(c, c->xs, indptr_host, indices_host, data_host, x_dtype, N, d, nnz, c->csr_densify_below);
    if (rc == DBGSOM_OK) rc = sync(c);
    if (rc != DBGSOM_OK) { (void)hipStreamSynchronize(c->stream); c->xs.dtype = -1; c->xs.csr = false; }
    else c->x_up((size_t)nnz * (4 + dtype_size(x_dtype)) + (size_t)(N + 1) * 8);
    return rc;
}

int dbgsom_ctx_load_device(dbgsom_ctx *c, const void *X_dev, int x_dtype, int64_t N, int64_t d, int64_t ldx) {
    CTX_CHECK(c);
    DBGSOM_REQUIRE(valid_dtype(x_dtype), "x_dtype must be DBGSOM_F32/F64/BF16");
    DBGSOM_REQUIRE(X_dev && N >= 1 && d >= 1 && ldx >= d && N < 0x7fffffff, "bad samples");
    reset_training_state(c);
    set_tight(c, false);
    Samples &s = c->xs;
    const int rc = place_device_samples(c, s, X_dev, x_dtype, N, d, ldx);
    if (rc != DBGSOM_OK) { (void)hipStreamSynchronize(c->stream); s.dtype = -1; return rc; }
    return sync(c);
}

int dbgsom_ctx_read_samples(dbgsom_ctx *c, const int64_t *rows_host, int64_t n, double *out_host) {
    CTX_CHECK(c);
    TRY(loaded(c, __func__));
    DBGSOM_REQUIRE(n >= 0 && (n == 0 || (rows_host && out_host)), "bad arguments");
    if (n == 0) return DBGSOM_OK;
    Samples &s = c->xs;
    for (int64_t r = 0; r < n; ++r) DBGSOM_REQUIRE(rows_host[r] >= 0 && rows_host[r] < s.N, "row index out of range");
// ... 1045 lines not shown
            hipLaunchKernelGGL(gather_i32_kernel, dim3(grid1d(n)), dim3(256), 0, c->stream, c->y.as<int32_t>(), order, first, n, k->y.as<int32_t>());
            if ((rc = launch_status("gather_i32_kernel"))) break;
            k->has_labels = true;
        }
        if (c->has_weights) {
            if ((rc = k->sw.reserve((size_t)n * 8))) break;
            hipLaunchKernelGGL(gather_f64_kernel, dim3(grid1d(n)), dim3(256), 0, c->stream, c->sw.as<double>(), order, first, n, k->sw.as<double>());
            if ((rc = launch_status("gather_f64_kernel"))) break;
            k->has_weights = true;
        }
        if ((rc = sync(c))) break;
        if ((rc = finish_samples(k, t, false))) break;
        rc = sync(k);
    } while (0);
    if (rc != DBGSOM_OK) { (void)hipStreamSynchronize(c->stream); dbgsom_ctx_destroy(k); return rc; }
    *child_out = k;
    return DBGSOM_OK;
}

int dbgsom_ctx_epoch_info(dbgsom_ctx *c, double *info8) {
    CTX_CHECK(c);
    DBGSOM_REQUIRE(info8, "null pointer");
    info8[0] = c->last_filtered ? 1.0 : 0.0;
    const SearchPolicy &pol = c->policy;
    info8[1] = pol.last_mean;
    info8[2] = c->last_filtered ? (double)pol.planes_used : 0.0;
    info8[3] = pol.last_hinted ? 1.0 : 0.0;
    info8[4] = (double)pol.filter_backoff;
    info8[5] = (double)pol.plane_hold;
    info8[6] = c->last_filtered && pol.last_probed ? pol.last_probe_mean : NAN;
    info8[7] = c->last_filtered && pol.last_seed_full ? 1.0 : 0.0;
    return DBGSOM_OK;
}

int dbgsom_ctx_arm_ms(dbgsom_ctx *c, double *ms12) {
    CTX_CHECK(c);
    DBGSOM_REQUIRE(ms12, "null pointer");
    for (int s_ = 0; s_ < 3; ++s_)
        for (int q = 0; q < 4; ++q) ms12[4 * s_ + q] = c->policy.arm_ms[s_][q];
    return DBGSOM_OK;
}

int dbgsom_ctx_filter_counts(dbgsom_ctx *c, uint32_t *counts_host, int64_t n) {
    CTX_CHECK(c);
    DBGSOM_REQUIRE(counts_host, "null pointer");
    if (!c->last_filter_ws) { set_error("dbgsom_ctx_filter_counts: no filtered search has run"); return DBGSOM_ESTATE; }
    return dbgsom_bmu_filtered_counts(c->last_filter_ws, c->last_filter_N, c->last_filter_d, c->last_filter_M, counts_host, n,
                                      c->stream);
}

int dbgsom_ctx_refine_counts(dbgsom_ctx *c, uint64_t *out4) {
    CTX_CHECK(c);
    DBGSOM_REQUIRE(out4, "null pointer");
    if (!c->last_filter_ws) { set_error("dbgsom_ctx_refine_counts: no filtered search has run"); return DBGSOM_ESTATE; }
    return dbgsom_bmu_filtered_refine_counts(c->last_filter_ws, c->last_filter_N, c->last_filter_d, c->last_filter_M, out4,
                                             c->stream);
}

int dbgsom_ctx_read_anchors(dbgsom_ctx *c, int64_t *n_anchors, double *anchors_host, int32_t *anchor_of_host,
                            int32_t *order_host, int32_t *aseed_host) {
    CTX_CHECK(c);
    TRY(loaded(c, __func__));
    TRY(complete_rows(c, __func__));
    Samples &s = c->xs;
    if (s.anchor_state != 1) { set_error("dbgsom_ctx_read_anchors: the resident samples have no anchor buckets"); return DBGSOM_ESTATE; }
    if (aseed_host && !(c->last_anchor_seeded && c->last_filter_ws)) {
        set_error("dbgsom_ctx_read_anchors: the last search was not seeded from the anchors");
        return DBGSOM_ESTATE;
    }
    const int64_t A = s.n_anchors;
    if (n_anchors) *n_anchors = A;
    if (anchors_host)
        DBGSOM_HIP_CHECK(hipMemcpyAsync(anchors_host, s.anchors.p, (size_t)A * s.dp * 8, hipMemcpyDeviceToHost, c->stream));
    if (anchor_of_host)
        DBGSOM_HIP_CHECK(hipMemcpyAsync(anchor_of_host, s.anchor_of.p, (size_t)s.N * 4, hipMemcpyDeviceToHost, c->stream));
    if (order_host)
        DBGSOM_HIP_CHECK(hipMemcpyAsync(order_host, s.anchor_order.p, (size_t)s.N * 4, hipMemcpyDeviceToHost, c->stream));
    if (aseed_host)
        return dbgsom_bmu_filtered_anchor_seeds(c->last_filter_ws, c->last_filter_N, c->last_filter_d, c->last_filter_M, (int)A,
                                                aseed_host, nullptr, c->stream);
    return sync(c);
}

int dbgsom_ctx_phase_ms(dbgsom_ctx *c, double *ms8) {
    CTX_CHECK(c);
    DBGSOM_REQUIRE(ms8, "null pointer");
    if (!c->timing || !c->ev_valid) { set_error("dbgsom_ctx_phase_ms: no timed epoch (set option \"timing\")"); return DBGSOM_ESTATE; }
    for (int k = 0; k < 3; ++k) {
        float ms = 0.f;
        DBGSOM_HIP_CHECK(hipEventElapsedTime(&ms, c->ev[k], c->ev[k + 1]));
        ms8[k] = ms;
    }
    for (int k = 0; k < 5; ++k) ms8[3 + k] = c->filter_ms_valid ? c->filter_ms[k] : 0.0;
    return DBGSOM_OK;
}

}
```

dbgsom_amd/csrc/filter.hip:

```cpp
#include <math.h>
#include <type_traits>

#include "bmu_common.h"
#include "filter_form.h"

namespace dbgsom {

constexpr double FQ = 8323072.0;
constexpr double F16 = 32512.0;
constexpr int FNT = 512;
constexpr int FSTAGES = 3;
constexpr int SCHED_BINS = 16;
constexpr int SCHED_RETRY = 2 * SCHED_BINS + 10;
constexpr int SCHED_CTR = 2 * SCHED_BINS + 12;
constexpr int SCHED_SUM = 2 * SCHED_BINS + 6;
constexpr int RF_CTR = 4;
static_assert(SCHED_CTR % 2 == 0, "the 64-bit counters of the refinement sit behind the schedule's");

__device__ __forceinline__ double plane16_residual(double r2, double s, double amax, int d) {
    (void)s;
    return sqrt(r2) * (1.0 + 1e-9 + 2.3e-16 * (double)d) + sqrt((double)d) * amax * 4e-16;
}

template <typename T>
// ... 1217 lines not shown
        const int rp = pb + b * 32 + lc, rj = jb + b * 32 + lc;
        base[0][b] = wt + (size_t)rp * FKT; sw[0][b] = (rp >> 2) & 3;
        base[1][b] = wt + (size_t)rj * FKT; sw[1][b] = (rj >> 2) & 3;
    }
    struct Fr { v4i_t v[2][NB]; };
    auto load = [&](int ks, Fr &f) {
        const size_t tile = (size_t)(ks >> 1) * w_rows * FKT;
        const int c = (ks & 1) * 2 + lh;
#pragma unroll
        for (int sd = 0; sd < 2; ++sd)
#pragma unroll
            for (int b = 0; b < NB; ++b)
                f.v[sd][b] = *reinterpret_cast<const v4i_t *>(base[sd][b] + tile + ((c ^ sw[sd][b]) << 4));
    };
    v16i_t P[NB][NB];
#pragma unroll
    for (int jt = 0; jt < NB; ++jt)
#pragma unroll
        for (int it = 0; it < NB; ++it)
#pragma unroll
            for (int r = 0; r < 16; ++r) P[jt][it][r] = 0;
    Fr f0, f1, f2, f3;
    load(0, f0);
    load(1, f1);
    for (int ks = 0; ks < nks; ks += 4) {
        if (ks + 2 < nks) { load(ks + 2, f2); load(ks + 3, f3); }
#pragma unroll
        for (int jt = 0; jt < NB; ++jt)
#pragma unroll
            for (int it = 0; it < NB; ++it) {
                P[jt][it] = __builtin_amdgcn_mfma_i32_32x32x32_i8(f0.v[1][jt], f0.v[0][it], P[jt][it], 0, 0, 0);
                P[jt][it] = __builtin_amdgcn_mfma_i32_32x32x32_i8(f1.v[1][jt], f1.v[0][it], P[jt][it], 0, 0, 0);
            }
        if (ks + 2 >= nks) break;
        if (ks + 4 < nks) { load(ks + 4, f0); load(ks + 5, f1); }
#pragma unroll
        for (int jt = 0; jt < NB; ++jt)
#pragma unroll
            for (int it = 0; it < NB; ++it) {
                P[jt][it] = __builtin_amdgcn_mfma_i32_32x32x32_i8(f2.v[1][jt], f2.v[0][it], P[jt][it], 0, 0, 0);
                P[jt][it] = __builtin_amdgcn_mfma_i32_32x32x32_i8(f3.v[1][jt], f3.v[0][it], P[jt][it], 0, 0, 0);
            }
    }
    const double root_d = sqrt((double)d) * (1.0 + 1e-12);
    __shared__ double tj_s[64], aj_s[64], ej_s[64];
    {
        const int j = jb + lane;
        const double tj = j < M ? tw[j] : 0.0;
        tj_s[lane] = tj;
        aj_s[lane] = gap_row_sq(tj, j < M ? wn0[j] + 0.0 * ww[j] : 0.0);
        ej_s[lane] = gap_row_err(root_d, tj);
    }
    __syncthreads();
#pragma unroll
    for (int it = 0; it < NB; ++it) {
        const int p = pb + it * 32 + lc;
        const bool pok = p < M;
        const double tp = pok ? tw[p] : 0.0, Ap = gap_row_sq(tp, pok ? wn0[p] + 0.0 * ww[p] : 0.0);
        const double ep = gap_row_err(root_d, tp);
        float near_ub = INFINITY;
#pragma unroll
        for (int jt = 0; jt < NB; ++jt)
#pragma unroll
            for (int r = 0; r < 16; ++r) {
                const int jl = jt * 32 + 4 * lh + (r & 3) + 8 * (r >> 2), j = jb + jl;
                if (!pok || j >= M) continue;
                const double tj = tj_s[jl], Pv = (double)P[jt][it][r];
                const double sq = __dadd_rn(Ap, aj_s[jl]), cr = 2.0 * tp * tj * Pv, epj = __dadd_rn(ep, ej_s[jl]);
                if (nnub && j != p) {
                    const double uh2 = ((sq - cr) + 1e-12 * (sq + fabs(cr))) * (1.0 / 16129.0) * (1.0 + 1e-12);
                    const double dh = uh2 > 0.0 ? sqrt(uh2) * (1.0 + 1e-12) : (uh2 == uh2 ? 0.0 : uh2);
                    const double ub = (dh + epj) * (1.0 + 1e-6);
                    if (ub < 3.0e38) near_ub = fminf(near_ub, __double2float_ru(ub));
                }
                const double dh2 = ((sq - cr) - 1e-12 * (sq + fabs(cr))) * (1.0 / 16129.0);
                const double lo = (dh2 > 0.0 ? sqrt(dh2) * (1.0 - 1e-12) : 0.0) - epj;
                const double v = lo > 0.0 ? lo * lo * (1.0 - 1e-6) : 0.0;
                gap[(size_t)j * ldg + p] = (v > 0.0 && v < 3.0e38) ? __double2float_rz(v) : 0.f;
            }
        if (nnub && pok && near_ub < INFINITY) atomicMin(&nnub[p], __float_as_uint(near_ub));
    }
}

__global__ __launch_bounds__(256, 6) void prune_mark_kernel(
    const int8_t *__restrict__ xplanes, const double *__restrict__ sx, const double *__restrict__ xx, int64_t N, int d,
    int dpad, const int8_t *__restrict__ wplanes, int w_rows, const double *__restrict__ tw,
    const double *__restrict__ ww, const double *__restrict__ summary, int M,
    const int64_t *__restrict__ prev, const int32_t *__restrict__ order, const float *__restrict__ gap, int ldg,
    uint16_t *__restrict__ ulist, int ulist_stride, uint32_t *__restrict__ ucount, uint32_t *__restrict__ sched_ctr,
    unsigned long long *__restrict__ sum_out, int count_only, const double *__restrict__ dist_prev,
    const double *__restrict__ shift, int32_t *__restrict__ retry_groups, unsigned long long *__restrict__ retry_len,
    int retry_mode, uint32_t retry_above, const uint32_t *__restrict__ nnub) {
    __shared__ int prev_s[128], run_p[128];
    __shared__ int64_t samp_s[128];
    __shared__ unsigned long long bound_s[128], run_t[128];
    __shared__ uint32_t mask[PRUNE_MAX_M / 32];
    __shared__ int misc[2];
    const int tid = threadIdx.x, lane = tid & 63, wave = tid >> 6;
    int64_t group = blockIdx.x;
    if (retry_mode == 2) {
        if ((unsigned long long)blockIdx.x >= *retry_len) return;
        group = retry_groups[blockIdx.x];
    }
    const int64_t p0 = group * 128;
    const int nwords = (M + 31) / 32;
    const unsigned long long INF_BITS = 0x7ff0000000000000ull;
    for (int w = tid; w < nwords; w += 256) mask[w] = 0u;
    if (tid < 128) {
        const int64_t p = p0 + tid;
        int pj = -2;
        int64_t i = 0;
        if (p < N) {
            i = (int64_t)order[p];
            const int64_t q = prev[i];
            pj = (q >= 0 && q < M) ? (int)q : -1;
        }
        prev_s[tid] = pj;
        samp_s[tid] = i;
        run_t[tid] = 0ull;
    }
    if (tid == 0) misc[0] = 0;
    __syncthreads();
    const double yy_max = summary[2], root_d = sqrt((double)d) * (1.0 + 1e-12);
    const int q = tid & 7, nch = dpad / 16;
    int a0r[4] = {0, 0, 0, 0}, axr[4] = {0, 0, 0, 0}, awr[4] = {0, 0, 0, 0};
    const int8_t *xrow[4], *wrow[4];
    int wswz[4], xodd = 0;
    bool live[4];
    double hint_up[4];
#pragma unroll
    for (int r = 0; r < 4; ++r) {
        const int il = r * 32 + (tid >> 3);
        const int pj = prev_s[il];
        hint_up[r] = -1.0;
        if (dist_prev && pj >= 0) {
            const double dp = dist_prev[samp_s[il]], sh = shift[pj];
            if (dp >= 0.0 && dp < INFINITY && sh >= 0.0 && sh <= 0.25 * dp) hint_up[r] = dp * (1.0 + 1e-7) + sh;
        }
        live[r] = pj >= 0 && !(hint_up[r] >= 0.0);
        xrow[r] = xplanes + (size_t)samp_s[il] * dpad;
        xodd |= (int)((((size_t)samp_s[il] * (size_t)dpad) >> 6) & 1) << r;
        wrow[r] = wplanes + (size_t)(live[r] ? pj : 0) * FKT;
        wswz[r] = live[r] ? (pj >> 2) & 3 : 0;
    }
#pragma unroll
    for (int rh = 0; rh < 4; rh += 2)
        for (int ch0 = q; ch0 < nch + 4; ch0 += 16) {
            v4i_t xv[2][2], wv[2][2];
#pragma unroll
            for (int r = 0; r < 2; ++r)
#pragma unroll
                for (int u = 0; u < 2; ++u) {
                    const int ch = ch0 + 8 * u - 4 * ((xodd >> (rh + r)) & 1);
                    const bool ok = live[rh + r] && ch >= 0 && ch < nch;
                    const v4i_t zero = {0, 0, 0, 0};
                    xv[r][u] = ok ? __builtin_nontemporal_load(reinterpret_cast<const v4i_t *>(xrow[rh + r] + ch * 16)) : zero;
                    wv[r][u] = ok ? *reinterpret_cast<const v4i_t *>(wrow[rh + r] + (size_t)(ch >> 2) * w_rows * FKT +
                                                                     (((ch & 3) ^ wswz[rh + r]) << 4)) : zero;
                }
#pragma unroll
            for (int r = 0; r < 2; ++r)
#pragma unroll
                for (int u = 0; u < 2; ++u)
#pragma unroll
                    for (int e = 0; e < 4; ++e) {
                        a0r[rh + r] = __builtin_amdgcn_sdot4(xv[r][u][e], wv[r][u][e], a0r[rh + r], false);
                        axr[rh + r] = __builtin_amdgcn_sdot4(xv[r][u][e], xv[r][u][e], axr[rh + r], false);
                        awr[rh + r] = __builtin_amdgcn_sdot4(wv[r][u][e], wv[r][u][e], awr[rh + r], false);
                    }
        }
#pragma unroll
    for (int round = 0; round < 4; ++round) {
#pragma unroll
        for (int m = 1; m < 8; m <<= 1) {
            a0r[round] += __shfl_xor(a0r[round], m, 64);
            axr[round] += __shfl_xor(axr[round], m, 64);
            awr[round] += __shfl_xor(awr[round], m, 64);
        }
    }
    {
        const int round = q & 3;
        const int il = round * 32 + (tid >> 3);
        const int pj = prev_s[il];
        const int64_t i = samp_s[il];
        const int a0 = round == 0 ? a0r[0] : (round == 1 ? a0r[1] : (round == 2 ? a0r[2] : a0r[3]));
        const int ax = round == 0 ? axr[0] : (round == 1 ? axr[1] : (round == 2 ? axr[2] : axr[3]));
        const int aw = round == 0 ? awr[0] : (round == 1 ? awr[1] : (round == 2 ? awr[2] : awr[3]));
        const double hint = round == 0 ? hint_up[0] : (round == 1 ? hint_up[1] : (round == 2 ? hint_up[2] : hint_up[3]));
        if (q < 4 && pj != -2) {
            unsigned long long bits = INF_BITS;
            if (pj >= 0) {
                const double sv = sx[i], tv = tw[pj];
                const double sq = sv * sv * (double)ax + tv * tv * (double)aw, cr = 2.0 * sv * tv * (double)a0;
                const double dh2 = ((sq - cr) + 1e-12 * (sq + fabs(cr))) / 16129.0;
                const double rho = 4.0 * (double)(d + 16) * 1.1102230246251565e-16 * (xx[i] + yy_max) + 0.0 * ww[pj];
                const double up = hint >= 0.0
                                      ? hint + sqrt(rho) * (1.0 + 1e-12)
                                      : (dh2 > 0.0 ? sqrt(dh2) * (1.0 + 1e-12) : 0.0) + root_d * (sv + tv) * PLANE0_ERR;
                if (fabs(up) < INFINITY) {
                    const double nn = nnub ? (double)__uint_as_float(nnub[pj]) : 0.0;
                    const double b = 2.0 * up * (1.0 + 1e-12) + nn * (1.0 + 1e-12) + (sqrt(2.0 * rho) * 1.0001 + 1e-300);
                    const double b2 = b * b * (1.0 + 1e-12);
                    if (b2 < INFINITY) bits = (unsigned long long)__double_as_longlong(b2);
                }
            }
            bound_s[il] = bits;
            if (bits == INF_BITS) misc[0] = 1;
        }
    }
    __syncthreads();
    const bool all = misc[0] != 0;
    if (!all) {
        if (wave == 0) {
            const int pa = prev_s[lane], pb_ = prev_s[lane + 64];
            const bool ha = pa != -2 && (lane == 0 || prev_s[lane - 1] != pa);
            const bool hb = pb_ != -2 && prev_s[lane + 63] != pb_;
            const uint64_t ba = __builtin_amdgcn_ballot_w64(ha), bb = __builtin_amdgcn_ballot_w64(hb);
            const uint64_t below = (lane == 63) ? ~0ull : ((1ull << (lane + 1)) - 1ull);
            const int ra = __popcll(ba & below) - 1, rb = __popcll(ba) + __popcll(bb & below) - 1;
            if (ha) run_p[ra] = pa;
            if (hb) run_p[rb] = pb_;
            if (pa != -2) atomicMax(&run_t[ra], bound_s[lane]);
            if (pb_ != -2) atomicMax(&run_t[rb], bound_s[lane + 64]);
            if (lane == 0) misc[1] = __popcll(ba) + __popcll(bb);
        }
        __syncthreads();
        const int nrun = misc[1];
        constexpr int JU = 4;
        for (int jb = wave * 64; jb < M; jb += 256 * JU) {
            bool keep[JU] = {false, false, false, false};
            for (int r = 0; r < nrun; r += 4) {
                int pr[4];
                double T[4];
#pragma unroll
                for (int v = 0; v < 4; ++v) {
                    const int rr = r + v < nrun ? r + v : r;
                    pr[v] = run_p[rr];
                    T[v] = __longlong_as_double((long long)run_t[rr]);
                }
                float g[JU][4];
#pragma unroll
                for (int u = 0; u < JU; ++u) {
                    const int j = jb + 256 * u + lane;
                    const int jc = j < M ? j : M - 1;
#pragma unroll
                    for (int v = 0; v < 4; ++v) g[u][v] = gap[(size_t)pr[v] * ldg + jc];
                }
#pragma unroll
                for (int u = 0; u < JU; ++u) {
                    const int j = jb + 256 * u + lane;
#pragma unroll
                    for (int v = 0; v < 4; ++v) keep[u] |= (j == pr[v]) || !((double)g[u][v] >= T[v]);
                }
            }
#pragma unroll
            for (int u = 0; u < JU; ++u) {
                const int j0 = jb + 256 * u;
                if (j0 >= M) break;
                const uint64_t b = __builtin_amdgcn_ballot_w64(keep[u] && j0 + lane < M);
                if (lane == 0) {
                    mask[j0 >> 5] = (uint32_t)b;
                    if ((j0 >> 5) + 1 < nwords) mask[(j0 >> 5) + 1] = (uint32_t)(b >> 32);
                }
            }
        }
    } else {
        for (int w = tid; w < nwords; w += 256) {
            const int left = M - w * 32;
            mask[w] = left >= 32 ? 0xffffffffu : ((1u << left) - 1u);
        }
    }
    __syncthreads();
    if (wave == 0) {
        const uint32_t base = compact_marked(mask, nwords, lane, ulist + (size_t)group * ulist_stride, !count_only);
        if (lane == 0) {
            if (retry_mode == 1 && base > retry_above) {
                retry_groups[atomicAdd(retry_len, 1ull)] = (int32_t)group;
            } else {
                if (retry_mode == 0 && base > retry_above) atomicAdd(retry_len, 1ull);
                if (!count_only) {
                    ucount[group] = base;
                    atomicAdd(&sched_ctr[sched_bin(base)], 1u);
                }
                atomicAdd(sum_out, (unsigned long long)base);
            }
        }
    }
}

typedef double ad4_t __attribute__((ext_vector_type(4)));
constexpr int ANCHOR_MAX = 256;
constexpr int ANCHOR_TICKET0 = 16;

__device__ __forceinline__ bool seed_less(double v, int j, double bv, int bj) { return v < bv || (v == bv && j < bj); }

__global__ __launch_bounds__(256) void anchor_seed_kernel(const double *__restrict__ anchors, int A,
                                                          const double *__restrict__ W, int M, int d,
                                                          const double *__restrict__ ww, double *__restrict__ part_val,
                                                          int32_t *__restrict__ part_idx, uint32_t *__restrict__ tickets,
                                                          int32_t *__restrict__ aseed) {
    __shared__ double val_s[4][16];
    __shared__ int idx_s[4][16];
    const int tid = threadIdx.x, lane = tid & 63, wave = tid >> 6, r = lane & 15, q = lane >> 4;
    const int npart = gridDim.x, ab = blockIdx.y * 16, jb = blockIdx.x * 64 + wave * 16;
    const int jrow = min(jb + r, M - 1), arow = min(ab + r, A - 1);
    const double *wp = W + (size_t)jrow * d + 4 * q, *ap = anchors + (size_t)arow * d + 4 * q;
    ad4_t c = {0.0, 0.0, 0.0, 0.0};
#pragma unroll 4
    for (int k = 0; k < d; k += 16) {
        const ad4_t wv = *reinterpret_cast<const ad4_t *>(wp + k), av = *reinterpret_cast<const ad4_t *>(ap + k);
        c = __builtin_amdgcn_mfma_f64_16x16x4f64(wv[0], av[0], c, 0, 0, 0);
        c = __builtin_amdgcn_mfma_f64_16x16x4f64(wv[1], av[1], c, 0, 0, 0);
        c = __builtin_amdgcn_mfma_f64_16x16x4f64(wv[2], av[2], c, 0, 0, 0);
        c = __builtin_amdgcn_mfma_f64_16x16x4f64(wv[3], av[3], c, 0, 0, 0);
    }
    double bv = INFINITY;
    int bj = 0x7fffffff;
#pragma unroll
    for (int u = 0; u < 4; ++u) {
        const int j = jb + 4 * u + q;
        if (j >= M) continue;
        const double y = ww[j], v = y - 2.0 * c[u];
        const double key = fabs(y) < INFINITY ? (fabs(v) < INFINITY ? v : 1.7976931348623157e308) : INFINITY;
        if (seed_less(key, j, bv, bj)) { bv = key; bj = j; }
    }
#pragma unroll
    for (int off = 16; off < 64; off <<= 1) {
        const double ov = __shfl_xor(bv, off, 64);
        const int oj = __shfl_xor(bj, off, 64);
        if (seed_less(ov, oj, bv, bj)) { bv = ov; bj = oj; }
    }
    if (q == 0) { val_s[wave][r] = bv; idx_s[wave][r] = bj; }
    __syncthreads();
    if (tid < 16 && ab + tid < A) {
        bv = val_s[0][tid]; bj = idx_s[0][tid];
#pragma unroll
        for (int w = 1; w < 4; ++w)
            if (seed_less(val_s[w][tid], idx_s[w][tid], bv, bj)) { bv = val_s[w][tid]; bj = idx_s[w][tid]; }
        part_val[(size_t)(ab + tid) * npart + blockIdx.x] = bv;
        part_idx[(size_t)(ab + tid) * npart + blockIdx.x] = bj;
    }
    if (!last_workgroup_done(tickets + ANCHOR_TICKET0 + blockIdx.y, (uint32_t)npart)) return;
    const int a = ab + (tid >> 4), sub = tid & 15;
    bv = INFINITY; bj = 0x7fffffff;
    if (a < A)
        for (int p = sub; p < npart; p += 16) {
            const double v = part_val[(size_t)a * npart + p];
            const int j = part_idx[(size_t)a * npart + p];
            if (seed_less(v, j, bv, bj)) { bv = v; bj = j; }
        }
#pragma unroll
    for (int off = 1; off < 16; off <<= 1) {
        const double ov = __shfl_xor(bv, off, 64);
        const int oj = __shfl_xor(bj, off, 64);
        if (seed_less(ov, oj, bv, bj)) { bv = ov; bj = oj; }
    }
    if (sub == 0 && a < A) aseed[a] = bj;
}

__global__ __launch_bounds__(256) void anchor_gather_kernel(const int32_t *__restrict__ aseed,
                                                            const int32_t *__restrict__ anchor_of, int64_t N,
                                                            int64_t *__restrict__ seed) {
    for (int64_t i = (int64_t)blockIdx.x * 256 + threadIdx.x; i < N; i += (int64_t)gridDim.x * 256)
        seed[i] = (int64_t)aseed[anchor_of[i]];
}

__global__ __launch_bounds__(256) void narrow_seeds_kernel(const int64_t *__restrict__ seed, int64_t N,
                                                           int32_t *__restrict__ out) {
    for (int64_t i = (int64_t)blockIdx.x * 256 + threadIdx.x; i < N; i += (int64_t)gridDim.x * 256)
        out[i] = (int32_t)seed[i];
// ... 515 lines not shown
    a.idx = idx_dev; a.dist = dist_dev; a.ws = workspace_dev; a.ws_bytes = workspace_bytes;
    a.stream = (hipStream_t)stream;
    a.refine_rows = (seed_stride & DBGSOM_REFINE) ? 192 : 0;
    return launch_bmu_filtered(a);
}

int dbgsom_bmu_filtered_anchored(const void *X_dev, int x_dtype, int64_t N, int64_t d, int64_t ldx,
                                 const double *xx_dev, const void *xplanes_dev, const double *W_dev,
                                 int64_t M, const double *ww_dev, const double *anchors_dev, int n_anchors,
                                 const int32_t *anchor_of_dev, const int32_t *order_dev, int seed_stride,
                                 int sweep_planes, int round_f32, int64_t *idx_dev, double *dist_dev,
                                 void *workspace_dev, size_t workspace_bytes, void *stream) {
    DBGSOM_REQUIRE(anchor_of_dev, "anchor seeds: null anchor_of");
    DBGSOM_REQUIRE(is_aligned(anchors_dev, 16), "alignment");
    FilteredCall a;
    a.X = X_dev; a.x_dtype = x_dtype; a.N = N; a.d = d; a.ldx = ldx; a.xx = xx_dev; a.xplanes = xplanes_dev;
    a.W = W_dev; a.M = M; a.ww = ww_dev; a.order = order_dev;
    a.anchors = anchors_dev; a.n_anchors = n_anchors; a.anchor_of = anchor_of_dev;
    a.seed_stride = seed_stride & ~DBGSOM_REFINE; a.sweep_planes = sweep_planes; a.round_f32 = round_f32;
    a.idx = idx_dev; a.dist = dist_dev; a.ws = workspace_dev; a.ws_bytes = workspace_bytes;
    a.stream = (hipStream_t)stream;
    a.refine_rows = (seed_stride & DBGSOM_REFINE) ? 192 : 0;
    return launch_bmu_filtered(a);
}

}

int dbgsom::filter_stage_ms(FilterAux &aux, double *ms5) {
    DBGSOM_REQUIRE(ms5, "null pointer");
    StageTimer &t = aux.timer;
    if (!t.enabled || !t.valid) { set_error("no timed dbgsom_bmu_filtered call"); return DBGSOM_ESTATE; }
    DBGSOM_HIP_CHECK(hipEventSynchronize(t.ev[5]));
    for (int k = 0; k < 5; ++k) {
        float ms = 0.f;
        DBGSOM_HIP_CHECK(hipEventElapsedTime(&ms, t.ev[k], t.ev[k + 1]));
        ms5[k] = ms;
    }
    return DBGSOM_OK;
}

namespace {
struct FilterRun {
    const FilteredCall &c;
    const FilterForm &fm;
    FilterAux &aux;
    hipStream_t s;
    int d, dpad;
    PlaneBuf xb;
    FilterWs f;
    const int64_t *seeds;
    const int32_t *order;
    bool gap_aside = false;

    unsigned long long *retry_len() const { return reinterpret_cast<unsigned long long *>(f.sched_ctr + SCHED_RETRY); }

    template <typename Kernel>
    void sweep_i8(Kernel kernel, bool seeding) const {
        const int32_t *no_sel = nullptr;
        hipLaunchKernelGGL(kernel, dim3((unsigned)f.nb), dim3(FNT), 0, s, xb.planes, xb.scale, xb.l1, c.xx, c.N, d, dpad,
                           seeding ? f.wt_sub : f.wt, seeding ? f.yy_sub : f.yctab, seeding ? f.ctab_sub : f.ictab,
                           seeding ? f.yy_sub : f.yypad, seeding ? f.ctab_sub : f.ctab, f.summary, seeding ? fm.Msub : (int)c.M,
                           seeding ? nullptr : seeds, seeding ? nullptr : order, f.ulist, (int)f.Mpad, f.ucount,
                           seeding ? f.seed : nullptr, seeding ? fm.seed_stride : 1, seeding ? fm.Msubpad : (int)f.Mpad,
                           seeding ? fm.nkt_used : 0, seeding ? f.kt_sel : no_sel, f.sched_ctr);
    }

    enum Sweep4Pass { PREPASS, RESEED, MARK };
    void sweep4(Sweep4Pass pass) const {
        const bool sub = pass == PREPASS, mark = pass == MARK, reseed = pass == RESEED;
        const float *tab = f.tab32 + (size_t)(mark ? 0 : (sub ? 2 : 4)) * f.Mpad;
        const int32_t *no_sel = nullptr, *retry = f.retry;
        hipLaunchKernelGGL(mark ? sweep4_i8_kernel<0> : sweep4_i8_kernel<1>, dim3((unsigned)f.nb), dim3(FNT), 0, s, xb.planes,
                           xb.scale, xb.l1, c.xx, c.N, d, dpad, sub ? f.wt_sub : f.wt, tab, tab + (size_t)f.Mpad,
                           sub ? f.yy_sub : f.yypad, sub ? f.ctab_sub : f.ctab, f.summary, sub ? fm.Msub : (int)c.M,
                           mark ? seeds : nullptr, sub ? nullptr : order, f.ulist, (int)f.Mpad, f.ucount,
                           mark ? nullptr : f.seed, sub ? fm.seed_stride : 1, sub ? fm.Msubpad : (int)f.Mpad,
                           sub ? fm.nkt_used : 0, sub ? f.kt_sel : no_sel, f.sched_ctr, f.chk32, reseed ? retry : no_sel,
                           reseed ? retry_len() : nullptr);
    }

    void prune_mark(int retry_mode, bool hinted) const {
        const bool hint = hinted && c.hint_shift;
        unsigned long long *sum = reinterpret_cast<unsigned long long *>(f.sched_ctr + SCHED_SUM) + (fm.prune ? 0 : 1);
        hipLaunchKernelGGL(prune_mark_kernel, dim3((unsigned)f.nb), dim3(256), 0, s, xb.planes, xb.scale, c.xx, c.N, d, dpad,
                           f.wt, (int)f.Mpad, f.wscale, c.ww, f.summary, (int)c.M, seeds, order, f.gap, (int)f.Mg, f.ulist,
                           (int)f.Mpad, f.ucount, f.sched_ctr, sum, fm.prune ? 0 : 1, hint ? c.hint_dist : nullptr,
                           hint ? c.hint_shift : nullptr, f.retry, retry_len(), retry_mode,
                           (uint32_t)(c.M / 8 > 96 ? c.M / 8 : 96), fm.k2 ? f.nnub : nullptr);
    }

    int gaps(hipStream_t gs) const {
        const unsigned gt = (unsigned)(f.Mg / 64);
        uint32_t *nnub = fm.k2 ? f.nnub : nullptr;
        if (nnub) DBGSOM_HIP_CHECK(hipMemsetAsync(nnub, 0x7f, (size_t)f.Mg * 4, gs));
        hipLaunchKernelGGL(fm.gap_nb == 2 ? proto_gap_kernel<2> : proto_gap_kernel<1>,
                           fm.gap_nb == 2 ? dim3(gt, gt) : dim3(2 * gt, 2 * gt), dim3(64), 0, gs, f.wt, (int)f.Mpad, dpad,
                           (int)c.M, d, f.wscale, f.wn0, c.ww, f.gap, (int)f.Mg, nnub);
        return DBGSOM_OK;
    }

    void prepare_prototypes() const {
        const bool select = fm.nkt_used < fm.nkt_full && !c.anchor_of;
        if (select) {
            hipLaunchKernelGGL(tile_partial_kernel, dim3((unsigned)fm.nkt_full, TS_RB), dim3(256), 0, s, c.W, (int)c.M, d,
                               dpad, f.tile_part);
            hipLaunchKernelGGL(tile_score_select_kernel, dim3((unsigned)fm.nkt_full), dim3(64), 0, s, f.tile_part, (int)c.M,
                               dpad, f.tile_score, fm.nkt_full, fm.nkt_used, f.kt_sel, f.tickets + 0);
        }
        WTables tables;
        tables.ww = c.ww; tables.ctab = f.ctab; tables.yypad = f.yypad; tables.ctab_sub = f.ctab_sub;
        tables.yy_sub = f.yy_sub; tables.ictab = f.ictab; tables.yctab = f.yctab; tables.summary = f.summary;
        tables.sched_ctr = f.sched_ctr; tables.tscale = sweep_tscale(fm.sweep_planes); tables.tab32 = f.tab32; tables.chk32 = f.chk32;
        hipLaunchKernelGGL(slice_w_tiled_kernel, dim3((unsigned)((c.M + 3) / 4)), dim3(256), 0, s, c.W, (int)c.M, d, dpad,
                           (int)f.Mpad, fm.seed_stride, fm.Msubpad, fm.nkt_used, select ? f.kt_sel : (const int32_t *)nullptr,
                           f.wt, f.wt_sub, f.wscale, f.wl1, f.yy_part, f.wn0, f.wres16, f.tickets + 1, tables);
    }

    int seed_and_sort() {
        if (seeds) {
            aux.timer.mark(2, s);
            return DBGSOM_OK;
        }
        if (c.anchor_of) return seed_from_anchors();
        SideStream &side = aux.side;
        if (fm.gap_nb && side.ready()) {
            DBGSOM_HIP_CHECK(hipEventRecord(side.gap_fork, s));
            DBGSOM_HIP_CHECK(hipStreamWaitEvent(side.stream, side.gap_fork, 0));
            const int rc = gaps(side.stream);
            if (rc != DBGSOM_OK) return rc;
            DBGSOM_HIP_CHECK(hipEventRecord(side.gap_done, side.stream));
            gap_aside = true;
        }
        if (fm.sweep_planes == 1) sweep4(PREPASS);
        else sweep_i8(sweep_i8_kernel<1, 2, 2>, true);
        aux.timer.mark(2, s);
        seeds = f.seed;
        order = f.order;
        if (c.seeds_out) {
            hipLaunchKernelGGL(narrow_seeds_kernel, dim3(seed_grid()), dim3(256), 0, s, f.seed, c.N, c.seeds_out);
            return launch_bucket_sort(f.seed, c.N, c.M, c.order_out, f.sort_ws, s);
        }
        return launch_bucket_sort(f.seed, c.N, c.M, f.order, f.sort_ws, s);
    }

    unsigned seed_grid() const { const int64_t g = (c.N + 255) / 256; return (unsigned)(g < 2048 ? g : 2048); }

    int seed_from_anchors() {
        SideStream &side = aux.side;
        if (fm.gap_nb && side.ready()) {
            DBGSOM_HIP_CHECK(hipEventRecord(side.gap_fork, s));
            DBGSOM_HIP_CHECK(hipStreamWaitEvent(side.stream, side.gap_fork, 0));
            const int rc = gaps(side.stream);
            if (rc != DBGSOM_OK) return rc;
            DBGSOM_HIP_CHECK(hipEventRecord(side.gap_done, side.stream));
            gap_aside = true;
        }
        hipLaunchKernelGGL(anchor_seed_kernel, dim3((unsigned)(f.Mg / 64), (unsigned)((c.n_anchors + 15) / 16)), dim3(256),
                           0, s, c.anchors, c.n_anchors, c.W, (int)c.M, d, c.ww, f.apart_val, f.apart_idx, f.tickets, f.aseed);
        hipLaunchKernelGGL(anchor_gather_kernel, dim3(seed_grid()), dim3(256), 0, s, f.aseed, c.anchor_of, c.N, f.seed);
        aux.timer.mark(2, s);
        seeds = f.seed;
        return DBGSOM_OK;
    }

    int mark_candidates() const {
        if (fm.gap_nb) {
            if (gap_aside) {
                DBGSOM_HIP_CHECK(hipStreamWaitEvent(s, aux.side.gap_done, 0));
            } else {
                const int rc = gaps(s);
                if (rc != DBGSOM_OK) return rc;
// ... 37 lines not shown
                               N, (int)M, f.cand, f.rbest, defer_M);
        else
            hipLaunchKernelGGL(sched_fill_kernel, fill_grid, dim3(256), 0, s, f.ucount, (int)f.nb, f.sched_ctr, f.sched,
                               (const uint8_t *)nullptr);
        if (fork) {
            DBGSOM_HIP_CHECK(hipEventRecord(side.forked, s));
            DBGSOM_HIP_CHECK(hipStreamWaitEvent(s2, side.forked, 0));
            DBGSOM_HIP_CHECK(hipStreamWaitEvent(s3, side.forked, 0));
        }
        if (refine) {
            hipLaunchKernelGGL(sched_fill_kernel, fill_grid, dim3(256), 0, s_mfma, f.ucount, (int)f.nb, f.sched_ctr, f.sched,
                               (const uint8_t *)f.gflag);
            if (fork) {
                DBGSOM_HIP_CHECK(hipEventRecord(side.mid, s_mfma));
                DBGSOM_HIP_CHECK(hipStreamWaitEvent(s3, side.mid, 0));
            }
            auto refine_launch = [&](auto kernel, int nj, int cls, int64_t wgs) {
                const int64_t nb8 = (f.nb + 7) / 8 * 8;
                hipLaunchKernelGGL(kernel, dim3((unsigned)(nb8 < wgs ? nb8 : wgs)), dim3(nj * 256), 0, s, xb.planes, xb.scale,
                                   xb.res16, c.xx, N, d, dpad, f.wt, (int)f.Mpad, f.wscale, c.ww, f.summary, order, f.ulist,
                                   (int)f.Mpad, f.ucount, f.rf_queue + (size_t)cls * f.nb, f.rf_qlen + cls, f.cand, f.rbest,
                                   f.rf_ctr, f.ovf, f.rf_qlen + 2, f.ovf_cand, defer_M, c.idx, c.dist);
            };
            if (fm.rows0 == 32) refine_launch(refine_i8_kernel<1, 1>, 1, 0, 1024);
            else if (fm.rows0 == 64) refine_launch(refine_i8_kernel<1, 2>, 1, 0, 1024);
            else if (fm.rows0 == 128) refine_launch(refine_i8_kernel<2, 2>, 2, 0, 512);
            refine_launch(refine_i8_kernel<2, 4>, 2, 1, 512);
            const int64_t Mk = defer_M ? M + 1 : M;
            const int rc = launch_bucket_sort(f.rbest, N, Mk, f.order2, f.sort_ws, s);
            if (rc != DBGSOM_OK) return rc;
            const uint32_t *n_active = defer_M ? bucket_sort_seg_start(f.sort_ws, N, Mk) + M : (const uint32_t *)nullptr;
            auto pair_launch = [&](auto kernel, auto *rows, int64_t ld) {
                const unsigned pgrid = (unsigned)(((N + PS - 1) / PS + 7) / 8 * 8);
                hipLaunchKernelGGL(kernel, dim3(pgrid), dim3(256), 0, s, rows, N, d, ld, c.xx, c.W, c.ww, f.order2, f.cand,
                                   c.round_f32, c.idx, c.dist, f.rf_ctr, n_active);
            };
            if (c.X_store && c.store_dtype == DBGSOM_BF16 && c.x_dtype == DBGSOM_F32)
                pair_launch(pair_exact_kernel<bf16_t, 32, 128>, (const bf16_t *)c.X_store, c.ld_store);
            else if (c.x_dtype == DBGSOM_F32) pair_launch(pair_exact_kernel<float, 16, 256>, (const float *)c.X, c.ldx);
            else pair_launch(pair_exact_kernel<double, 16, 256>, (const double *)c.X, c.ldx);
        }
        auto exact_stage = [&](auto xt) {
            using XT = decltype(xt);
            constexpr int XS = (int)sizeof(XT);
            const XT *X = (const XT *)c.X;
            if (refine)
                hipLaunchKernelGGL((overflow_exact_kernel<XT>), dim3(512), dim3(256), 0, s, X, d, c.ldx, c.xx, c.W, c.ww, f.ulist,
                                   (int)f.Mpad, f.ucount, f.ovf, f.rf_qlen + 2, f.ovf_cand, c.round_f32, c.idx, c.dist);
            auto launch = [&](auto kernel, dim3 grid, dim3 block, hipStream_t st) {
                hipLaunchKernelGGL(kernel, grid, block, 0, st, X, N, d, c.ldx, c.xx, c.W, (int)M, c.ww, order, f.ulist,
                                   (int)f.Mpad, f.ucount, f.sched, f.sched_ctr + 2 * SCHED_BINS, c.round_f32, c.idx, c.dist);
            };
            const unsigned nb = (unsigned)f.nb;
            switch (fm.exact) {
            case FilterForm::EXACT_K2:
                launch(subset_exact_kernel<XT, 3, 8, 1, 2>, dim3(nb), dim3(512), s_mfma);
                launch(subset_exact_kernel<XT, 2, 8, 1, 2>, dim3(nb), dim3(512), s2);
                launch(subset_exact_kernel<XT, 1, 8, 1, 2>, dim3(nb), dim3(512), s3);
                break;
            case FilterForm::EXACT_BESIDE_REFINE:
                launch(subset_exact_kernel<XT, 3, 4, 2, 1, split_ring_stages(3, XS)>, dim3(2 * nb), dim3(256), s_mfma);
                launch(subset_exact_kernel<XT, 2, 4, 2, 1, split_ring_stages(2, XS)>, dim3(2 * nb), dim3(256), s3);
                launch(subset_exact_kernel<XT, 1, 4, 2, 1, split_ring_stages(1, XS)>, dim3(2 * nb), dim3(256), s3);
                break;
            case FilterForm::EXACT_SPLIT:
                launch(subset_exact_split_kernel<XT>, dim3(2 * nb, 3), dim3(256), s);
                break;
            case FilterForm::EXACT_ALL: launch(subset_exact_all_kernel<XT>, dim3(nb), dim3(512), s); break;
            }
        };
        if (c.x_dtype == DBGSOM_F32) exact_stage(float{});
        else exact_stage(double{});
        if (fork) {
            DBGSOM_HIP_CHECK(hipEventRecord(side.joined, s2));
            DBGSOM_HIP_CHECK(hipEventRecord(side.joined2, s3));
            DBGSOM_HIP_CHECK(hipStreamWaitEvent(s, side.joined, 0));
            DBGSOM_HIP_CHECK(hipStreamWaitEvent(s, side.joined2, 0));
        }
        return DBGSOM_OK;
    }
};
}

int dbgsom::launch_bmu_filtered(const FilteredCall &call) {
    FilterForm form;
    const char *rejected = form.resolve(call.seed_stride, call.sweep_planes, call.k, call.refine_rows, call.defer_dist, call.N,
                                        call.d, call.M, call.prev_idx != nullptr);
    DBGSOM_REQUIRE(!rejected, rejected);
    DBGSOM_REQUIRE(call.x_dtype == DBGSOM_F32 || call.x_dtype == DBGSOM_F64, "the filtered search takes float32 or float64 samples");
    DBGSOM_REQUIRE(call.N >= 1 && call.N < 0x7fffffff && call.d >= 1 && call.d % KT == 0 && call.ldx >= call.d,
                   "bad sample shape (d must be a multiple of 16)");
    DBGSOM_REQUIRE(call.M >= 1 && call.M <= SW_MAX_M, "M outside [1, 16000]");
    const bool seeds_only = call.seeds_out != nullptr;
    DBGSOM_REQUIRE(call.X && call.xx && call.xplanes && call.W && call.ww && call.ws, "null pointer");
    DBGSOM_REQUIRE(seeds_only || (call.idx && call.dist), "null pointer");
    DBGSOM_REQUIRE(!seeds_only || (call.order_out && !call.prev_idx && !call.anchor_of && call.k == 1),
                   "seeds_out comes with order_out, on a stateless k = 1 call");
    DBGSOM_REQUIRE(!call.anchor_of || (call.anchors && call.order && !call.prev_idx && call.n_anchors >= 1 &&
                                       call.n_anchors <= ANCHOR_MAX && form.prune && !form.seed_full && call.k == 1),
                   "anchor seeds: the stateless k = 1 pruning form, with the anchors and the bucket order");
    DBGSOM_REQUIRE(call.anchor_of || (call.prev_idx == nullptr) == (call.order == nullptr),
                   "prev_idx and order come as a pair (both NULL = stateless two-pass search)");
    DBGSOM_REQUIRE(is_aligned(call.X, 16) && (call.ldx * (int64_t)dtype_size(call.x_dtype)) % 16 == 0 &&
                       is_aligned(call.W, 16) && is_aligned(call.ws, 256) && is_aligned(call.xplanes, 256), "alignment");
    if (call.ws_bytes < dbgsom_bmu_filtered_workspace_bytes(call.N, call.d, call.M)) {
        set_error("dbgsom_bmu_filtered: workspace too small");
        return DBGSOM_ENOMEM;
    }
    FilterAux &aux = call.aux ? *call.aux : g_aux;
    FilterRun r{call, form, aux, call.stream, (int)call.d, (int)filter_dpad(call.d), {}, {}, call.prev_idx, call.order};
    carve_planes(&r.xb, (char *)const_cast<void *>(call.xplanes), call.N, call.d);
    carve_filter(&r.f, (char *)call.ws, call.N, call.d, call.M);
    StageTimer &timer = aux.timer;
    timer.mark(0, r.s);
    r.prepare_prototypes();
    timer.mark(1, r.s);
    int rc = r.seed_and_sort();
    if (rc != DBGSOM_OK) return rc;
    if (seeds_only) return launch_status("seed pre-pass and bucket sort");
    timer.mark(3, r.s);
    rc = r.mark_candidates();
    if (rc != DBGSOM_OK) return rc;
    timer.mark(4, r.s);
    rc = call.guard_mean > 0.0 ? r.guard_lists() : DBGSOM_OK;
    if (rc == DBGSOM_OK) rc = r.exact_on_candidates();
    if (rc != DBGSOM_OK && rc != DBGSOM_LISTS_LONG) return rc;
    timer.mark(5, r.s);
    timer.valid = timer.enabled;
    return rc == DBGSOM_LISTS_LONG ? rc : launch_status("filtered bmu kernels");
}

extern "C" {


const unsigned long long *dbgsom_filter_count_sum_ptr(const void *workspace_dev, int64_t N, int64_t d, int64_t M) {
    FilterWs f;
    carve_filter(&f, (char *)const_cast<void *>(workspace_dev), N, d, M);
    return reinterpret_cast<const unsigned long long *>(f.sched_ctr + SCHED_SUM);
}

int dbgsom_bmu_filtered_refine_counts(const void *workspace_dev, int64_t N, int64_t d, int64_t M,
                                      uint64_t *out4, void *stream) {
    DBGSOM_REQUIRE(workspace_dev && out4, "null pointer");
    FilterWs f;
    carve_filter(&f, (char *)const_cast<void *>(workspace_dev), N, d, M);
    DBGSOM_HIP_CHECK(hipMemcpyAsync(out4, f.rf_ctr, (size_t)RF_CTR * 8, hipMemcpyDeviceToHost, (hipStream_t)stream));
    DBGSOM_HIP_CHECK(hipStreamSynchronize((hipStream_t)stream));
    return DBGSOM_OK;
}

int dbgsom_bmu_filtered_counts_async(const void *workspace_dev, int64_t N, int64_t d, int64_t M,
                                     uint32_t *counts_host, int64_t n_counts, void *stream) {
    DBGSOM_REQUIRE(workspace_dev && counts_host, "null pointer");
    FilterWs f;
    carve_filter(&f, (char *)const_cast<void *>(workspace_dev), N, d, M);
    DBGSOM_REQUIRE(n_counts == f.nb, "n_counts must be ceil(N / 128)");
    DBGSOM_HIP_CHECK(hipMemcpyAsync(counts_host, f.ucount, (size_t)f.nb * 4, hipMemcpyDeviceToHost,
                                    (hipStream_t)stream));
    return DBGSOM_OK;
}

int dbgsom_bmu_filtered_counts(const void *workspace_dev, int64_t N, int64_t d, int64_t M,
                               uint32_t *counts_host, int64_t n_counts, void *stream) {
    const int rc = dbgsom_bmu_filtered_counts_async(workspace_dev, N, d, M, counts_host, n_counts, stream);
    if (rc != DBGSOM_OK) return rc;
    DBGSOM_HIP_CHECK(hipStreamSynchronize((hipStream_t)stream));
    return DBGSOM_OK;
}

int dbgsom_bmu_filtered_gaps(const void *workspace_dev, int64_t N, int64_t d, int64_t M, float *gap_host, void *stream) {
    DBGSOM_REQUIRE(workspace_dev && gap_host, "null pointer");
    DBGSOM_REQUIRE(N >= 1 && d >= 1 && M >= 1 && M <= PRUNE_MAX_M, "no gap table: M outside [1, 8192]");
    FilterWs f;
    carve_filter(&f, (char *)const_cast<void *>(workspace_dev), N, d, M);
    DBGSOM_HIP_CHECK(hipMemcpy2DAsync(gap_host, (size_t)M * 4, f.gap, (size_t)f.Mg * 4, (size_t)M * 4, (size_t)M,
                                      hipMemcpyDeviceToHost, (hipStream_t)stream));
    DBGSOM_HIP_CHECK(hipStreamSynchronize((hipStream_t)stream));
    return DBGSOM_OK;
}

int dbgsom_bmu_filtered_anchor_seeds(const void *workspace_dev, int64_t N, int64_t d, int64_t M, int n_anchors,
                                     int32_t *aseed_host, int64_t *seed_host, void *stream) {
    DBGSOM_REQUIRE(workspace_dev && aseed_host, "null pointer");
    DBGSOM_REQUIRE(N >= 1 && d >= 1 && M >= 1 && M <= PRUNE_MAX_M, "no anchor seeds: M outside [1, 8192]");
    DBGSOM_REQUIRE(n_anchors >= 1 && n_anchors <= ANCHOR_MAX, "n_anchors outside [1, 256]");
    FilterWs f;
    carve_filter(&f, (char *)const_cast<void *>(workspace_dev), N, d, M);
    DBGSOM_HIP_CHECK(hipMemcpyAsync(aseed_host, f.aseed, (size_t)n_anchors * 4, hipMemcpyDeviceToHost, (hipStream_t)stream));
    if (seed_host)
        DBGSOM_HIP_CHECK(hipMemcpyAsync(seed_host, f.seed, (size_t)N * 8, hipMemcpyDeviceToHost, (hipStream_t)stream));
    DBGSOM_HIP_CHECK(hipStreamSynchronize((hipStream_t)stream));
    return DBGSOM_OK;
}

}
```

dbgsom_amd/csrc/filter_form.h:

```cpp
#pragma once

#include <stdint.h>

#include "../../include/dbgsom_hip.h"

namespace dbgsom {

constexpr int FKT = 64;
constexpr int PREPASS_KTILES = 3;
constexpr int SW_MAX_KT = 1024;
constexpr int PRUNE_MAX_M = 8192;
constexpr int SWEEP4_MAX_M = 8192;

inline int64_t filter_dpad(int64_t d) {
    const int64_t p = (d + FKT - 1) / FKT * FKT;
    return p < 2 * FKT ? 2 * FKT : p;
}

struct __attribute__((visibility("hidden"))) FilterForm {
    bool seed_full = false;
    bool prune = false, prune_probe = false;
    bool prune_retry = false;
    bool k2 = false;
    int seed_stride = 0, Msub = 0, Msubpad = 0, nkt_full = 0, nkt_used = 0;
    int sweep_planes = 0;
    enum Marking {
        MARK_PRUNE,
        MARK_SWEEP4,
        MARK_SWEEP_1_4,
        MARK_SWEEP_2_2,
        MARK_SWEEP_3_1
    } marking = MARK_SWEEP_2_2;
    int gap_nb = 0;
    bool refine = false;
    int rows0 = 0;
    enum Exact {
        EXACT_K2,
        EXACT_BESIDE_REFINE,
        EXACT_SPLIT,
        EXACT_ALL
    } exact = EXACT_ALL;

    const char *resolve(int flags, int planes, int k, int refine_rows, bool defer, int64_t N, int64_t d, int64_t M,
                        bool has_hint) {
        seed_full = (flags & DBGSOM_SEED_FULL) != 0;
        prune = (flags & DBGSOM_PRUNE) != 0 && M <= PRUNE_MAX_M;
        prune_probe = !prune && (flags & DBGSOM_PRUNE_PROBE) != 0 && M <= PRUNE_MAX_M;
        prune_retry = (flags & DBGSOM_PRUNE_RETRY) != 0 && !seed_full && !has_hint;
        k2 = k == 2;
        if (!(k == 1 || k == 2)) return "k must be 1 or 2";
        if (!(!defer || (refine_rows > 0 && M < 0xffff))) return "deferred distances need the refinement";
        if (!(!k2 || (prune && refine_rows == 0 && M >= 2)))
            return "k = 2 needs the pruning form (DBGSOM_PRUNE, M <= 8192) without the refinement";
        seed_stride = flags & ~(DBGSOM_PRUNE | DBGSOM_PRUNE_PROBE | DBGSOM_PRUNE_RETRY);
        seed_stride = seed_full ? 1 : seed_stride;
        if (!(seed_stride >= 0 && seed_stride <= 64)) return "seed_stride outside [0, 64]";
        if (!(planes >= 0 && planes <= 3)) return "sweep_planes must be 0 .. 3";
        sweep_planes = planes == 0 ? 2 : planes;
        if (seed_stride == 0) {
            seed_stride = (int)((M + 255) / 256);
            seed_stride = seed_stride < 4 ? 4 : (seed_stride > 64 ? 64 : seed_stride);
        }
        while (seed_stride > 1 && (M + seed_stride - 1) / seed_stride < 128) seed_stride >>= 1;
        Msub = (int)((M + seed_stride - 1) / seed_stride);
        Msubpad = (Msub + 255) / 256 * 256;
        nkt_full = (int)filter_dpad(d) / FKT;
        nkt_used = (!seed_full && PREPASS_KTILES < nkt_full && nkt_full <= SW_MAX_KT) ? PREPASS_KTILES : nkt_full;
        if (prune) marking = MARK_PRUNE;
        else if (sweep_planes == 1) marking = M <= SWEEP4_MAX_M ? MARK_SWEEP4 : MARK_SWEEP_1_4;
        else marking = sweep_planes == 3 ? MARK_SWEEP_3_1 : MARK_SWEEP_2_2;
        const int64_t gt = ((M + 63) / 64 * 64) / 64;
        gap_nb = (prune || prune_probe) ? (gt * gt >= 1024 ? 2 : 1) : 0;
        refine = refine_rows > 0;
        rows0 = refine_rows <= 32 ? 32 : (refine_rows <= 64 ? 64 : (refine_rows <= 128 ? 128 : 0));
        const int64_t nb = (N + 127) / 128;
        exact = k2 ? EXACT_K2 : (refine ? EXACT_BESIDE_REFINE : (nb <= 1024 ? EXACT_SPLIT : EXACT_ALL));
        return nullptr;
    }
};

}
```

include/dbgsom_hip.h:

```cpp
#ifndef DBGSOM_HIP_H
#define DBGSOM_HIP_H

#include <stddef.h>
#include <stdint.h>

#ifdef __cplusplus
extern "C" {
#endif

#define DBGSOM_ABI_VERSION 4

#define DBGSOM_F32 0
#define DBGSOM_F64 1
#define DBGSOM_BF16 2

#define DBGSOM_CENTRES_COMPACT 0
#define DBGSOM_CENTRES_ALIGNED 1

#define DBGSOM_OK 0
#define DBGSOM_EINVAL (-1)
#define DBGSOM_EHIP (-2)
#define DBGSOM_ENOMEM (-3)
#define DBGSOM_ESTATE (-4)
#define DBGSOM_ERANGE (-5)
#define DBGSOM_ECALLBACK (-6)

#define DBGSOM_SEED_FULL 0x100
#define DBGSOM_PRUNE 0x200
#define DBGSOM_PRUNE_PROBE 0x400
#define DBGSOM_PRUNE_RETRY 0x800
#define DBGSOM_REFINE 0x1000

#define DBGSOM_MAX_PROTOTYPES 16000

int dbgsom_abi_version(void);
const char *dbgsom_last_error(void);
int dbgsom_device_count(int *count);


int dbgsom_row_sqnorms(const void *A_dev, int dtype, int64_t rows, int64_t d, int64_t ld,
                       double *out_dev, void *stream);

int dbgsom_bmu(const void *X_dev, int x_dtype, int64_t N, int64_t d, int64_t ldx,
               const double *xx_dev, const double *W_dev, int64_t M, const double *ww_dev, int k,
               int round_f32, int64_t *idx_dev, double *dist_dev, void *stream);

int dbgsom_exp_similarity(const double *dist_dev, int64_t N, double gamma, double *kw_dev,
                          void *stream);

size_t dbgsom_accumulate_workspace_bytes(int64_t N, int64_t d, int64_t M);
int dbgsom_accumulate(const void *X_dev, int x_dtype, int64_t N, int64_t d, int64_t ldx,
                      const int64_t *idx_dev, const double *kw_dev, const double *dist_dev,
                      int64_t M, double *sums_dev, int32_t *status_dev, void *workspace_dev,
                      size_t workspace_bytes, void *stream);

size_t dbgsom_accumulate_weighted_workspace_bytes(int64_t N, int64_t d, int64_t M);
int dbgsom_accumulate_weighted(const void *X_dev, int x_dtype, int64_t N, int64_t d, int64_t ldx,
                               const int64_t *idx_dev, const double *kw_dev, const double *sw_dev,
                               const double *dist_dev, int64_t M, double *sums_dev, int32_t *status_dev,
                               void *workspace_dev, size_t workspace_bytes, void *stream);

int dbgsom_csr_check(const int64_t *indptr_host, const int32_t *indices_host, int64_t N, int64_t d, int64_t nnz);
int dbgsom_csr_row_sqnorms(const int64_t *indptr_dev, const void *data_dev, int x_dtype, int64_t N, double *out_dev,
                           void *stream);
int64_t dbgsom_csr_wt_ld(int64_t M);
int dbgsom_csr_transpose_weights(const double *W_dev, int64_t M, int64_t d, int64_t ldw, double *Wt_dev, int64_t ldwt,
                                 void *stream);
int dbgsom_bmu_csr(const int64_t *indptr_dev, const int32_t *indices_dev, const void *data_dev, int x_dtype, int64_t N,
                   const double *xx_dev, const double *Wt_dev, int64_t ldwt, int64_t M, const double *ww_dev, int k,
                   int round_f32, int64_t *idx_dev, double *dist_dev, void *stream);
int dbgsom_csr_densify(const int64_t *indptr_dev, const int32_t *indices_dev, const void *data_dev, int x_dtype,
                       int64_t N, int64_t d, int64_t ld, void *out_dev, void *stream);
size_t dbgsom_accumulate_csr_workspace_bytes(int64_t N, int64_t d, int64_t M);
int dbgsom_accumulate_csr(const int64_t *indptr_dev, const int32_t *indices_dev, const void *data_dev, int x_dtype,
                          int64_t N, int64_t d, const int64_t *idx_dev, const double *kw_dev, const double *sw_dev,
                          const double *dist_dev, int64_t M, double *sums_dev, int32_t *status_dev,
                          void *workspace_dev, size_t workspace_bytes, void *stream);

size_t dbgsom_smooth_workspace_bytes(int64_t M, int64_t d);
int dbgsom_smooth(const double *sums_dev, int64_t M, int64_t d, const float *hop_dev,
                  double sigma, int layout, const double *W_old_dev, double *W_new_dev,
                  double *change_total_dev, void *workspace_dev, size_t workspace_bytes,
                  void *stream);

size_t dbgsom_filter_planes_bytes(int64_t rows, int64_t d);
int dbgsom_filter_prepare(const void *X_dev, int x_dtype, int64_t N, int64_t d, int64_t ldx,
                          void *planes_dev, size_t planes_bytes, void *stream);
size_t dbgsom_bmu_filtered_workspace_bytes(int64_t N, int64_t d, int64_t M);
int dbgsom_bmu_filtered(const void *X_dev, int x_dtype, int64_t N, int64_t d, int64_t ldx,
                        const double *xx_dev, const void *xplanes_dev, const double *W_dev,
                        int64_t M, const double *ww_dev, const int64_t *prev_idx_dev,
                        const int32_t *order_dev, int seed_stride, int sweep_planes,
                        int round_f32, int64_t *idx_dev, double *dist_dev, void *workspace_dev,
                        size_t workspace_bytes, void *stream);
int dbgsom_filter_timing(int enable);
int dbgsom_bmu_filtered_stage_ms(double *ms5);
int dbgsom_bmu_filtered_counts(const void *workspace_dev, int64_t N, int64_t d, int64_t M,
                               uint32_t *counts_host, int64_t n_counts, void *stream);
int dbgsom_bmu_filtered_counts_async(const void *workspace_dev, int64_t N, int64_t d, int64_t M,
                                     uint32_t *counts_host, int64_t n_counts, void *stream);
int dbgsom_bmu_filtered_gaps(const void *workspace_dev, int64_t N, int64_t d, int64_t M, float *gap_host,
                             void *stream);
int dbgsom_bmu_filtered_anchored(const void *X_dev, int x_dtype, int64_t N, int64_t d, int64_t ldx,
                                 const double *xx_dev, const void *xplanes_dev, const double *W_dev,
                                 int64_t M, const double *ww_dev, const double *anchors_dev, int n_anchors,
                                 const int32_t *anchor_of_dev, const int32_t *order_dev, int seed_stride,
                                 int sweep_planes, int round_f32, int64_t *idx_dev, double *dist_dev,
                                 void *workspace_dev, size_t workspace_bytes, void *stream);
int dbgsom_bmu_filtered_anchor_seeds(const void *workspace_dev, int64_t N, int64_t d, int64_t M, int n_anchors,
                                     int32_t *aseed_host, int64_t *seed_host, void *stream);

int dbgsom_bmu_filtered_refine_counts(const void *workspace_dev, int64_t N, int64_t d, int64_t M,
                                      uint64_t *out4, void *stream);


size_t dbgsom_sum_workspace_bytes(void);
int dbgsom_sum_f64(const double *v_dev, int64_t n, double *out_dev, void *workspace_dev,
                   size_t workspace_bytes, void *stream);

int dbgsom_topographic_count(const int64_t *idx2_dev, int64_t n, const int32_t *xy_dev, int64_t M,
                             uint64_t *count_dev, void *stream);

int dbgsom_column_sums(const void *X_dev, int x_dtype, int64_t N, int64_t d, int64_t ldx,
                       const void *mean_dev, void *out_dev, void *stream);

int dbgsom_density_terms(const double *dist_dev, int64_t n, double sigma, double *out_dev,
                         void *stream);

int dbgsom_weighted_sum_f64(const double *v_dev, const double *w_dev, int64_t n, double *out_dev,
                            void *workspace_dev, size_t workspace_bytes, void *stream);
int dbgsom_topographic_weight(const int64_t *idx2_dev, const double *w_dev, int64_t n, const int32_t *xy_dev,
                              int64_t M, double *out_dev, void *workspace_dev, size_t workspace_bytes,
                              void *stream);
int dbgsom_class_histogram_weighted(const int32_t *order_dev, const uint32_t *seg_start_dev, const int32_t *y_dev,
                                    const double *w_dev, int64_t n, int64_t M, int64_t n_classes,
                                    double *hist_dev, void *stream);
size_t dbgsom_weighted_column_sums_workspace_bytes(int64_t d);
int dbgsom_weighted_column_sums(const void *X_dev, int x_dtype, int64_t N, int64_t d, int64_t ldx,
                                const double *w_dev, const double *mean_dev, double *out_dev,
                                void *workspace_dev, size_t workspace_bytes, void *stream);

int dbgsom_class_histogram(const int64_t *idx_dev, const int32_t *y_dev, int64_t n, int64_t M,
                           int64_t n_classes, uint64_t *hist_dev, void *stream);

typedef struct dbgsom_ctx dbgsom_ctx;

#define DBGSOM_ALG_AUTO 0
#define DBGSOM_ALG_EXACT 1
#define DBGSOM_ALG_FILTERED 2
#define DBGSOM_ALG_FILTERED_HINT 3

#define DBGSOM_EPOCH_FROZEN 1

int dbgsom_ctx_create(int device, dbgsom_ctx **out);
int dbgsom_ctx_destroy(dbgsom_ctx *ctx);

int dbgsom_ctx_set_option(dbgsom_ctx *ctx, const char *name, int64_t value);
int dbgsom_ctx_get_option(dbgsom_ctx *ctx, const char *name, int64_t *value);
int dbgsom_ctx_stream(dbgsom_ctx *ctx, void **stream);

int dbgsom_ctx_load(dbgsom_ctx *ctx, const void *X_host, int x_dtype, int64_t N, int64_t d,
                    int storage);
int dbgsom_ctx_load_csr(dbgsom_ctx *ctx, const int64_t *indptr_host, const int32_t *indices_host,
                        const void *data_host, int x_dtype, int64_t N, int64_t d, int64_t nnz);
int dbgsom_ctx_load_device(dbgsom_ctx *ctx, const void *X_dev, int x_dtype, int64_t N, int64_t d,
                           int64_t ldx);
int dbgsom_ctx_read_samples(dbgsom_ctx *ctx, const int64_t *rows_host, int64_t n, double *out_host);
int dbgsom_ctx_set_labels(dbgsom_ctx *ctx, const int32_t *y_host, int64_t N);
int dbgsom_ctx_set_sample_weight(dbgsom_ctx *ctx, const double *w_host, int64_t N);
int dbgsom_ctx_weight_total(dbgsom_ctx *ctx, double *out_host);
int dbgsom_ctx_weighted_column_sums(dbgsom_ctx *ctx, const double *mean_host, double *out_host);
int dbgsom_ctx_class_histogram_weighted(dbgsom_ctx *ctx, const int64_t *idx_host, int64_t n_classes, int64_t M,
                                        double *hist_host);

int dbgsom_ctx_set_topology(dbgsom_ctx *ctx, const double *hop_host, int64_t M);

typedef int (*dbgsom_allreduce_fn)(void *user, double *buf_dev, int64_t count, void *stream);
int dbgsom_ctx_set_allreduce(dbgsom_ctx *ctx, dbgsom_allreduce_fn fn, void *user);
int dbgsom_rccl_unique_id(char *id128);
int dbgsom_rccl_comm_init(const char *id128, int nranks, int rank, void **comm_out);
int dbgsom_rccl_comm_destroy(void *comm);
int dbgsom_ctx_set_rccl(dbgsom_ctx *ctx, void *nccl_comm);
enum { DBGSOM_COLL_ALLREDUCE = 0, DBGSOM_COLL_REDUCE_SCATTER = 1, DBGSOM_COLL_ALLGATHER = 2 };
typedef int (*dbgsom_collective_fn)(void *user, int op, double *buf_dev, int64_t count, void *stream);
int dbgsom_ctx_set_collectives(dbgsom_ctx *ctx, dbgsom_collective_fn fn, void *user, int rank, int nranks);
// ... 34 lines not shown
size_t dbgsom_accumulate_masked_workspace_bytes(int64_t N, int64_t d, int64_t M);
int dbgsom_accumulate_masked(const void *X_dev, int x_dtype, int64_t N, int64_t d, int64_t ldx,
                             const int64_t *idx_dev, const double *kw_dev, const double *dist_dev, int64_t M,
                             double *sums_dev, int32_t *status_dev, void *workspace_dev, size_t workspace_bytes,
                             void *stream);
size_t dbgsom_smooth_masked_workspace_bytes(int64_t M, int64_t d);
int dbgsom_smooth_masked(const double *sums_dev, int64_t M, int64_t d, const float *hop_dev, double sigma,
                         const double *W_old_dev, double *W_new_dev, double *change_total_dev,
                         void *workspace_dev, size_t workspace_bytes, void *stream);
int dbgsom_ctx_bmu_masked(dbgsom_ctx *ctx, const double *W_host, int64_t M, int k, int64_t *idx_host,
                          double *dist_host);
int dbgsom_ctx_epoch_masked(dbgsom_ctx *ctx, const double *W_host, int64_t M, double gamma, double sigma,
                            double *W_new_host, double *change_total_host, double *errors_host,
                            double *activations_host, int64_t *idx_host, double *dist_host);

#define DBGSOM_SC_COUNTS 11
size_t dbgsom_sparse_code_workspace_bytes(int64_t Nq, int64_t d, int64_t M, int max_iter);
int dbgsom_sparse_code(const void *Xq_dev, int x_dtype, int64_t Nq, int64_t d, int64_t ldx,
                       const double *W_dev, int64_t M, int64_t ldw, int max_iter, int cap,
                       const double *P_dev, int64_t C, double *code_dev, double *proba_dev,
                       uint64_t *counts_dev, void *workspace_dev, size_t workspace_bytes,
                       void *stream);
int dbgsom_sparse_code_timing(int enable);
int dbgsom_sparse_code_stage_ms(double *ms5);
int dbgsom_ctx_sparse_code(dbgsom_ctx *ctx, const void *Xq_host, int x_dtype, int64_t Nq, int64_t d,
                           const double *W_host, int64_t M, int max_iter, const double *P_host,
                           int64_t C, double *code_host, double *proba_host, uint64_t *counts_host);
int dbgsom_ctx_sparse_code_device(dbgsom_ctx *ctx, const void *Xq_dev, int x_dtype, int64_t Nq, int64_t d,
                                  int64_t ldx, const double *W_host, int64_t M, int max_iter,
                                  const double *P_host, int64_t C, double *code_dev, double *proba_dev,
                                  uint64_t *counts_host);

size_t dbgsom_topofn_workspace_bytes(int64_t M, int full);
int dbgsom_topofn(const int64_t *idx2_dev, int64_t n, const int32_t *xy_dev, int64_t M, int64_t n_pos,
                  uint64_t *hist_pos_dev, uint64_t *hist_neg_dev, int32_t *D_dev, void *ws,
                  size_t ws_bytes, void *stream);
int dbgsom_topofn_timing(int enable);
int dbgsom_topofn_stage_ms(double *ms4);
int dbgsom_ctx_topographic_function(dbgsom_ctx *ctx, const void *Xq_host, int x_dtype, int64_t Nq,
                                    int64_t d, const double *W_host, int64_t M, int round_f32,
                                    const int32_t *xy_host, int64_t n_pos, int64_t *hist_pos_host,
                                    int64_t *hist_neg_host, int32_t *D_host);
int dbgsom_ctx_topographic_function_device(dbgsom_ctx *ctx, const void *Xq_dev, int x_dtype, int64_t Nq,
                                           int64_t d, int64_t ldx, const double *W_host, int64_t M,
                                           int round_f32, const int32_t *xy_host, int64_t n_pos,
                                           int64_t *hist_pos_host, int64_t *hist_neg_host, int32_t *D_host);

int dbgsom_ctx_exp_similarity(dbgsom_ctx *ctx, const double *dist_host, int64_t n, double gamma,
                              double *kw_host);

int dbgsom_ctx_epoch(dbgsom_ctx *ctx, const double *W_host, int64_t M, int round_f32,
                     double gamma, double sigma, int layout, int flags, double *W_new_host,
                     double *change_total_host, double *errors_host, double *activations_host,
                     int64_t *idx_host, double *dist_host);

int dbgsom_ctx_update(dbgsom_ctx *ctx, const double *W_host, int64_t M, const int64_t *idx_host,
                      const double *kw_host, const double *dist_host, double sigma, int layout,
                      double *W_new_host, double *change_total_host, double *errors_host,
                      double *activations_host);

int dbgsom_ctx_set_hint(dbgsom_ctx *ctx, const int64_t *idx_host, int64_t M);

int dbgsom_ctx_read_sums(dbgsom_ctx *ctx, double *sums_host, int64_t M);

int dbgsom_ctx_column_sums(dbgsom_ctx *ctx, const void *mean_host, void *out_host);
int dbgsom_ctx_quantization_error(dbgsom_ctx *ctx, const double *W_host, int64_t M, int round_f32,
                                  double *out2_host);
int dbgsom_ctx_topographic_count(dbgsom_ctx *ctx, const double *W_host, int64_t M, int round_f32,
                                 const int32_t *xy_host, double *count_host);
int dbgsom_ctx_node_statistics(dbgsom_ctx *ctx, const double *W_host, int64_t M, int round_f32,
                               double sigma, double *hits_host, double *density_host);
int dbgsom_ctx_class_histogram(dbgsom_ctx *ctx, const int64_t *idx_host, int64_t n_classes,
                               int64_t M, int64_t *hist_host);

int dbgsom_ctx_partition(dbgsom_ctx *ctx, const double *W_host, int64_t M, int round_f32,
                         int64_t *counts_host, int64_t *idx_host);
int dbgsom_ctx_subset_create(dbgsom_ctx *ctx, int64_t neuron, dbgsom_ctx **child);

int dbgsom_ctx_epoch_info(dbgsom_ctx *ctx, double *info8);
int dbgsom_ctx_arm_ms(dbgsom_ctx *ctx, double *ms12);
int dbgsom_ctx_filter_counts(dbgsom_ctx *ctx, uint32_t *counts_host, int64_t n);
int dbgsom_ctx_read_anchors(dbgsom_ctx *ctx, int64_t *n_anchors, double *anchors_host, int32_t *anchor_of_host,
                            int32_t *order_host, int32_t *aseed_host);
int dbgsom_ctx_refine_counts(dbgsom_ctx *ctx, uint64_t *out4);
int dbgsom_ctx_phase_ms(dbgsom_ctx *ctx, double *ms8);

#ifdef __cplusplus
}
#endif
#endif
```

Before: 491.2 million samples/s/epoch.

## Cache bucket-ordered int8 plane with precomputed norms for anchor-seeded pruning

Builds, once per resident sample set, a copy of the first digit plane reordered into anchor-bucket order, together with each row's int8 self-dot norm. The prune-mark kernel then reads sample rows contiguously from that copy and takes x and w norms from precomputed tables, so it no longer recomputes two of its three sdot4 accumulations or their shuffles. The aim is to cut scattered gathers and ALU work in the hot prune pass. The cost is an extra N*dpad byte buffer, a one-time reorder kernel, and a changed chunk-swizzle path for odd-aligned rows.

```diff
diff --git a/dbgsom_amd/_native.py b/dbgsom_amd/_native.py
--- a/dbgsom_amd/_native.py
+++ b/dbgsom_amd/_native.py
@@ -50,6 +50,7 @@
     "dbgsom_bmu_filtered_counts_async": (_ci, [_vp, _i64, _i64, _i64, _vp, _i64, _vp]),
     "dbgsom_bmu_filtered_refine_counts": (_ci, [_vp, _i64, _i64, _i64, _vp, _vp]),
     "dbgsom_bmu_filtered_gaps": (_ci, [_vp, _i64, _i64, _i64, _vp, _vp]),
+    "dbgsom_bmu_filtered_lists": (_ci, [_vp, _i64, _i64, _i64, _vp, _i64, _vp]),
     "dbgsom_bmu_filtered_anchored": (_ci, [_vp, _ci, _i64, _i64, _i64, _vp, _vp, _vp, _i64, _vp, _vp, _ci, _vp, _vp,
                                            _ci, _ci, _ci, _vp, _vp, _vp, _sz, _vp]),
     "dbgsom_bmu_filtered_anchor_seeds": (_ci, [_vp, _i64, _i64, _i64, _ci, _vp, _vp, _vp]),
@@ -150,6 +151,8 @@
     "dbgsom_ctx_epoch_info": (_ci, [_vp, _vp]),
     "dbgsom_ctx_arm_ms": (_ci, [_vp, _vp]),
     "dbgsom_ctx_filter_counts": (_ci, [_vp, _vp, _i64]),
+    "dbgsom_ctx_filter_lists": (_ci, [_vp, _vp, _i64]),
+    "dbgsom_ctx_read_bucket_plane": (_ci, [_vp, _ci, ctypes.POINTER(_i64), _vp, _vp]),
     "dbgsom_ctx_read_anchors": (_ci, [_vp, ctypes.POINTER(_i64), _vp, _vp, _vp, _vp]),
     "dbgsom_ctx_refine_counts": (_ci, [_vp, _vp]),
     "dbgsom_ctx_phase_ms": (_ci, [_vp, _vp]),
diff --git a/dbgsom_amd/backend.py b/dbgsom_amd/backend.py
--- a/dbgsom_amd/backend.py
+++ b/dbgsom_amd/backend.py
@@ -359,6 +359,7 @@
     resident_csr = property(lambda self: bool(self._get("resident_csr")))
     planes_cached = property(lambda self: bool(self._get("planes_cached")))
     anchor_seeds = property(lambda self: self._get("anchor_seeds"), lambda self, v: self._set("anchor_seeds", int(v)))
+    bucket_plane = property(lambda self: self._get("bucket_plane"), lambda self, v: self._set("bucket_plane", int(v)))
     anchor_builds = property(lambda self: self._get("anchor_builds"))
     anchor_searches = property(lambda self: self._get("anchor_searches"))
     anchor_state = property(lambda self: self._get("anchor_state"))
@@ -900,6 +901,22 @@
         self._call("dbgsom_ctx_filter_counts", self._ctx, out.ctypes.data, nb)
         return out
 
+    def filter_lists(self, M):
+        nb = (self._N + 127) // 128
+        rows = np.empty((nb, int(M)), dtype=np.uint16)
+        self._call("dbgsom_ctx_filter_lists", self._ctx, rows.ctypes.data, nb)
+        return [rows[g, :n].copy() for g, n in enumerate(self.filter_counts())]
+
+    def read_bucket_plane(self, natural=False):
+        pitch = ctypes.c_int64(0)
+        self._call("dbgsom_ctx_read_bucket_plane", self._ctx, int(bool(natural)), ctypes.byref(pitch), None, None)
+        out = {"pitch": pitch.value, "plane": np.empty((self._N, pitch.value), dtype=np.int8)}
+        if not natural:
+            out["ax"] = np.empty(self._N, dtype=np.int32)
+        self._call("dbgsom_ctx_read_bucket_plane", self._ctx, int(bool(natural)), None, out["plane"].ctypes.data,
+                   None if natural else out["ax"].ctypes.data)
+        return out
+
     def read_anchors(self, aseed=False):
         n = ctypes.c_int64(0)
         self._call("dbgsom_ctx_read_anchors", self._ctx, ctypes.byref(n), None, None, None, None)
@@ -1043,7 +1060,8 @@
         return sub
 
     _SETTABLE = ("algorithm", "sweep_planes", "seed_stride", "timing", "graph", "refine", "defer",
-                 "filter_min_query_rows", "max_mean_candidates", "shard_smooth", "csr_densify_below", "anchor_seeds")
+                 "filter_min_query_rows", "max_mean_candidates", "shard_smooth", "csr_densify_below", "anchor_seeds",
+                 "bucket_plane")
 
     def release(self):
         if self._ctx:
diff --git a/dbgsom_amd/csrc/common.h b/dbgsom_amd/csrc/common.h
--- a/dbgsom_amd/csrc/common.h
+++ b/dbgsom_amd/csrc/common.h
@@ -232,11 +232,16 @@
     const double *anchors = nullptr;
     const int32_t *anchor_of = nullptr;
     int n_anchors = 0;
+    const int8_t *plane0_bucket = nullptr;
+    const int32_t *bucket_ax = nullptr;
+    int64_t bucket_pitch = 0;
     int32_t *seeds_out = nullptr, *order_out = nullptr;
     FilterAux *aux = nullptr;
 };
 constexpr int DBGSOM_LISTS_LONG = 1000;
 int launch_bmu_filtered(const FilteredCall &call);
+int launch_bucket_plane(const void *xplanes, int64_t N, int64_t d, const int32_t *order, int64_t pitch, int8_t *plane0_bucket,
+                        int32_t *bucket_ax, hipStream_t s);
 size_t smooth_workspace_bytes(int64_t M, int64_t d);
 int launch_smooth(const double *sums, int64_t M, int64_t d, const float *hop, double sigma,
                   int layout, const double *W_old, double *W_new, double *change_total, void *ws,
diff --git a/dbgsom_amd/csrc/engine.hip b/dbgsom_amd/csrc/engine.hip
--- a/dbgsom_amd/csrc/engine.hip
+++ b/dbgsom_amd/csrc/engine.hip
@@ -9,6 +9,7 @@
 
 #include "anchor_chain.h"
 #include "common.h"
+#include "filter_form.h"
 #include "search_policy.h"
 
 namespace dbgsom {
@@ -193,10 +194,14 @@
     DevBuf own, x32, xx, planes;
     bool planes_ready = false;
     DevBuf anchors, anchor_of, anchor_order;
+    DevBuf plane0_bucket, ax_bucket;
+    int64_t bucket_pitch = 0;
     int64_t n_anchors = 0;
     int anchor_state = 0;
+    void drop_bucket_plane() { plane0_bucket.release(); ax_bucket.release(); bucket_pitch = 0; }
     void drop_anchors(int state) {
         anchors.release(); anchor_of.release(); anchor_order.release();
+        drop_bucket_plane();
         n_anchors = 0; anchor_state = state;
     }
     void drop_planes() { planes_ready = false; drop_anchors(0); }
@@ -283,6 +288,7 @@
     bool filter_ms_valid = false;
     FilterAux faux;
     int anchor_seeds = 1;
+    int bucket_plane = 1;
     int64_t anchor_builds = 0, anchor_searches = 0;
     bool anchors_built_now = false;
     bool last_anchor_seeded = false;
@@ -443,8 +449,19 @@
     return DBGSOM_OK;
 }
 
+int ensure_bucket_plane(dbgsom_ctx *c, Samples &s) {
+    if (s.anchor_state != 1 || s.plane0_bucket.p) return DBGSOM_OK;
+    const int64_t pitch = bucket_plane_pitch(s.dp);
+    s.plane0_bucket.tight = s.ax_bucket.tight = true;
+    TRY(s.plane0_bucket.reserve((size_t)s.N * pitch));
+    TRY(s.ax_bucket.reserve((size_t)s.N * 4));
+    s.bucket_pitch = pitch;
+    return launch_bucket_plane(s.planes.p, s.N, s.dp, s.anchor_order.as<int32_t>(), pitch, s.plane0_bucket.as<int8_t>(),
+                               s.ax_bucket.as<int32_t>(), c->stream);
+}
+
 int ensure_anchors(dbgsom_ctx *c, Samples &s) {
-    if (s.anchor_state != 0) return DBGSOM_OK;
+    if (s.anchor_state != 0) return c->bucket_plane ? ensure_bucket_plane(c, s) : DBGSOM_OK;
     TRY(ensure_planes(c, s));
     const int64_t A = s.N < 256 ? s.N : 256, dp = s.dp;
     TRY(s.anchors.reserve((size_t)A * dp * 8 + (size_t)A * 8));
@@ -480,7 +497,7 @@
     s.anchor_state = 1;
     ++c->anchor_builds;
     c->anchors_built_now = true;
-    return DBGSOM_OK;
+    return c->bucket_plane ? ensure_bucket_plane(c, s) : DBGSOM_OK;
 }
 
 bool filter_shape_ok(const Samples &s, int64_t M) { return SearchPolicy::shape_ok(M, s.N, s.dp); }
@@ -538,6 +555,10 @@
         ++c->anchor_searches;
         call.anchors = s.anchors.as<double>(); call.n_anchors = (int)s.n_anchors;
         call.anchor_of = s.anchor_of.as<int32_t>(); call.order = s.anchor_order.as<int32_t>();
+        if (c->bucket_plane && s.plane0_bucket.p) {
+            call.plane0_bucket = s.plane0_bucket.as<int8_t>(); call.bucket_ax = s.ax_bucket.as<int32_t>();
+            call.bucket_pitch = s.bucket_pitch;
+        }
         c->last_anchor_seeded = true;
     }
     call.round_f32 = round_f32; call.idx = idx; call.dist = dist; call.ws = ws.p; call.ws_bytes = ws.cap;
@@ -1089,6 +1110,13 @@
     } else if (!strcmp(name, "anchor_seeds")) {
         DBGSOM_REQUIRE(v == 0 || v == 1, "anchor_seeds must be 0 or 1");
         c->anchor_seeds = (int)v;
+    } else if (!strcmp(name, "bucket_plane")) {
+        DBGSOM_REQUIRE(v == 0 || v == 1, "bucket_plane must be 0 or 1");
+        c->bucket_plane = (int)v;
+        if (!v) {
+            TRY(sync(c));
+            c->xs.drop_bucket_plane(); c->xq.drop_bucket_plane();
+        }
     } else if (!strcmp(name, "incomplete")) {
         DBGSOM_REQUIRE(v == 0 || v == 1, "incomplete must be 0 or 1");
         c->incomplete = false;
@@ -1144,6 +1172,7 @@
     else if (!strcmp(name, "prototypes")) *v = c->M;
     else if (!strcmp(name, "planes_cached")) *v = c->xs.planes_ready ? 1 : 0;
     else if (!strcmp(name, "anchor_seeds")) *v = c->anchor_seeds;
+    else if (!strcmp(name, "bucket_plane")) *v = c->bucket_plane;
     else if (!strcmp(name, "incomplete")) *v = c->incomplete ? 1 : 0;
     else if (!strcmp(name, "anchor_builds")) *v = c->anchor_builds;
     else if (!strcmp(name, "anchor_searches")) *v = c->anchor_searches;
@@ -1168,7 +1197,7 @@
         size_t tot = 0;
         for (const Samples *q : {&c->xs, &c->xq})
             tot += q->own.cap + q->x32.cap + q->xx.cap + q->planes.cap + q->indptr.cap + q->indices.cap + q->data.cap +
-                   q->anchors.cap + q->anchor_of.cap + q->anchor_order.cap;
+                   q->anchors.cap + q->anchor_of.cap + q->anchor_order.cap + q->plane0_bucket.cap + q->ax_bucket.cap;
         DevBuf *bufs[] = CTX_DEVBUFS(c);
         for (DevBuf *b : bufs) tot += b->cap;
         *v = (int64_t)tot;
@@ -2380,6 +2409,36 @@
     return sync(c);
 }
 
+int dbgsom_ctx_read_bucket_plane(dbgsom_ctx *c, int natural, int64_t *pitch, int8_t *plane_host, int32_t *ax_host) {
+    CTX_CHECK(c);
+    TRY(loaded(c, __func__));
+    Samples &s = c->xs;
+    if (natural) {
+        if (s.csr || !s.planes_ready) { set_error("dbgsom_ctx_read_bucket_plane: the resident samples have no digit planes"); return DBGSOM_ESTATE; }
+        if (pitch) *pitch = filter_dpad(s.dp);
+        if (plane_host)
+            DBGSOM_HIP_CHECK(hipMemcpyAsync(plane_host, s.planes.p, (size_t)s.N * filter_dpad(s.dp), hipMemcpyDeviceToHost, c->stream));
+        return sync(c);
+    }
+    if (s.anchor_state != 1 || !s.plane0_bucket.p) {
+        set_error("dbgsom_ctx_read_bucket_plane: the resident samples have no bucket-ordered plane");
+        return DBGSOM_ESTATE;
+    }
+    if (pitch) *pitch = s.bucket_pitch;
+    if (plane_host)
+        DBGSOM_HIP_CHECK(hipMemcpyAsync(plane_host, s.plane0_bucket.p, (size_t)s.N * s.bucket_pitch, hipMemcpyDeviceToHost, c->stream));
+    if (ax_host) DBGSOM_HIP_CHECK(hipMemcpyAsync(ax_host, s.ax_bucket.p, (size_t)s.N * 4, hipMemcpyDeviceToHost, c->stream));
+    return sync(c);
+}
+
+int dbgsom_ctx_filter_lists(dbgsom_ctx *c, uint16_t *lists_host, int64_t n_groups) {
+    CTX_CHECK(c);
+    DBGSOM_REQUIRE(lists_host, "null pointer");
+    if (!c->last_filter_ws) { set_error("dbgsom_ctx_filter_lists: no filtered search has run"); return DBGSOM_ESTATE; }
+    return dbgsom_bmu_filtered_lists(c->last_filter_ws, c->last_filter_N, c->last_filter_d, c->last_filter_M, lists_host,
+                                     n_groups, c->stream);
+}
+
 int dbgsom_ctx_phase_ms(dbgsom_ctx *c, double *ms8) {
     CTX_CHECK(c);
     DBGSOM_REQUIRE(ms8, "null pointer");
diff --git a/dbgsom_amd/csrc/filter.hip b/dbgsom_amd/csrc/filter.hip
--- a/dbgsom_amd/csrc/filter.hip
+++ b/dbgsom_amd/csrc/filter.hip
@@ -1323,6 +1323,7 @@
     }
 }
 
+template <bool BUCKET>
 __global__ __launch_bounds__(256, 6) void prune_mark_kernel(
     const int8_t *__restrict__ xplanes, const double *__restrict__ sx, const double *__restrict__ xx, int64_t N, int d,
     int dpad, const int8_t *__restrict__ wplanes, int w_rows, const double *__restrict__ tw,
@@ -1331,7 +1332,8 @@
     uint16_t *__restrict__ ulist, int ulist_stride, uint32_t *__restrict__ ucount, uint32_t *__restrict__ sched_ctr,
     unsigned long long *__restrict__ sum_out, int count_only, const double *__restrict__ dist_prev,
     const double *__restrict__ shift, int32_t *__restrict__ retry_groups, unsigned long long *__restrict__ retry_len,
-    int retry_mode, uint32_t retry_above, const uint32_t *__restrict__ nnub) {
+    int retry_mode, uint32_t retry_above, const uint32_t *__restrict__ nnub, const double *__restrict__ wn0,
+    const int8_t *__restrict__ xbucket, int pitch, const int32_t *__restrict__ ax_bucket) {
     __shared__ int prev_s[128], run_p[128];
     __shared__ int64_t samp_s[128];
     __shared__ unsigned long long bound_s[128], run_t[128];
@@ -1364,7 +1366,7 @@
     __syncthreads();
     const double yy_max = summary[2], root_d = sqrt((double)d) * (1.0 + 1e-12);
     const int q = tid & 7, nch = dpad / 16;
-    int a0r[4] = {0, 0, 0, 0}, axr[4] = {0, 0, 0, 0}, awr[4] = {0, 0, 0, 0};
+    int a0r[4] = {0, 0, 0, 0}, axr[4] = {0, 0, 0, 0};
     const int8_t *xrow[4], *wrow[4];
     int wswz[4], xodd = 0;
     bool live[4];
@@ -1379,8 +1381,9 @@
             if (dp >= 0.0 && dp < INFINITY && sh >= 0.0 && sh <= 0.25 * dp) hint_up[r] = dp * (1.0 + 1e-7) + sh;
         }
         live[r] = pj >= 0 && !(hint_up[r] >= 0.0);
-        xrow[r] = xplanes + (size_t)samp_s[il] * dpad;
-        xodd |= (int)((((size_t)samp_s[il] * (size_t)dpad) >> 6) & 1) << r;
+        const size_t xoff = BUCKET ? (size_t)(p0 + il) * (size_t)pitch : (size_t)samp_s[il] * (size_t)dpad;
+        xrow[r] = (BUCKET ? xbucket : xplanes) + xoff;
+        xodd |= (int)((xoff >> 6) & 1) << r;
         wrow[r] = wplanes + (size_t)(live[r] ? pj : 0) * FKT;
         wswz[r] = live[r] ? (pj >> 2) & 3 : 0;
     }
@@ -1392,7 +1395,8 @@
             for (int r = 0; r < 2; ++r)
 #pragma unroll
                 for (int u = 0; u < 2; ++u) {
-                    const int ch = ch0 + 8 * u - 4 * ((xodd >> (rh + r)) & 1);
+                    const bool odd = (xodd >> (rh + r)) & 1;
+                    const int ch = BUCKET && odd ? nch - 8 - ch0 - 8 * u + 2 * q : ch0 + 8 * u - 4 * (int)odd;
                     const bool ok = live[rh + r] && ch >= 0 && ch < nch;
                     const v4i_t zero = {0, 0, 0, 0};
                     xv[r][u] = ok ? __builtin_nontemporal_load(reinterpret_cast<const v4i_t *>(xrow[rh + r] + ch * 16)) : zero;
@@ -1406,8 +1410,8 @@
 #pragma unroll
                     for (int e = 0; e < 4; ++e) {
                         a0r[rh + r] = __builtin_amdgcn_sdot4(xv[r][u][e], wv[r][u][e], a0r[rh + r], false);
-                        axr[rh + r] = __builtin_amdgcn_sdot4(xv[r][u][e], xv[r][u][e], axr[rh + r], false);
-                        awr[rh + r] = __builtin_amdgcn_sdot4(wv[r][u][e], wv[r][u][e], awr[rh + r], false);
+                        if constexpr (!BUCKET)
+                            axr[rh + r] = __builtin_amdgcn_sdot4(xv[r][u][e], xv[r][u][e], axr[rh + r], false);
                     }
         }
 #pragma unroll
@@ -1415,8 +1419,7 @@
 #pragma unroll
         for (int m = 1; m < 8; m <<= 1) {
             a0r[round] += __shfl_xor(a0r[round], m, 64);
-            axr[round] += __shfl_xor(axr[round], m, 64);
-            awr[round] += __shfl_xor(awr[round], m, 64);
+            if constexpr (!BUCKET) axr[round] += __shfl_xor(axr[round], m, 64);
         }
     }
     {
@@ -1425,14 +1428,14 @@
         const int pj = prev_s[il];
         const int64_t i = samp_s[il];
         const int a0 = round == 0 ? a0r[0] : (round == 1 ? a0r[1] : (round == 2 ? a0r[2] : a0r[3]));
-        const int ax = round == 0 ? axr[0] : (round == 1 ? axr[1] : (round == 2 ? axr[2] : axr[3]));
-        const int aw = round == 0 ? awr[0] : (round == 1 ? awr[1] : (round == 2 ? awr[2] : awr[3]));
+        int ax = round == 0 ? axr[0] : (round == 1 ? axr[1] : (round == 2 ? axr[2] : axr[3]));
         const double hint = round == 0 ? hint_up[0] : (round == 1 ? hint_up[1] : (round == 2 ? hint_up[2] : hint_up[3]));
         if (q < 4 && pj != -2) {
             unsigned long long bits = INF_BITS;
             if (pj >= 0) {
                 const double sv = sx[i], tv = tw[pj];
-                const double sq = sv * sv * (double)ax + tv * tv * (double)aw, cr = 2.0 * sv * tv * (double)a0;
+                if constexpr (BUCKET) ax = ax_bucket[p0 + il];
+                const double sq = sv * sv * (double)ax + tv * tv * wn0[pj], cr = 2.0 * sv * tv * (double)a0;
                 const double dh2 = ((sq - cr) + 1e-12 * (sq + fabs(cr))) / 16129.0;
                 const double rho = 4.0 * (double)(d + 16) * 1.1102230246251565e-16 * (xx[i] + yy_max) + 0.0 * ww[pj];
                 const double up = hint >= 0.0
@@ -1527,6 +1530,26 @@
             }
         }
     }
+}
+
+__global__ __launch_bounds__(256) void bucket_plane_kernel(const int8_t *__restrict__ plane0, int dpad,
+                                                           const int32_t *__restrict__ order, int64_t N, int pitch,
+                                                           int8_t *__restrict__ out, int32_t *__restrict__ ax) {
+    const int lane = threadIdx.x & 63;
+    const int64_t p = (int64_t)blockIdx.x * 4 + (threadIdx.x >> 6);
+    if (p >= N) return;
+    const int8_t *src = plane0 + (size_t)order[p] * dpad;
+    int8_t *dst = out + (size_t)p * pitch;
+    int a = 0;
+    for (int ch = lane; ch < pitch / 16; ch += 64) {
+        v4i_t v = {0, 0, 0, 0};
+        if (ch < dpad / 16) v = __builtin_nontemporal_load(reinterpret_cast<const v4i_t *>(src + ch * 16));
+#pragma unroll
+        for (int e = 0; e < 4; ++e) a = __builtin_amdgcn_sdot4(v[e], v[e], a, false);
+        *reinterpret_cast<v4i_t *>(dst + ch * 16) = v;
+    }
+    for (int off = 32; off > 0; off >>= 1) a += __shfl_xor(a, off, 64);
+    if (lane == 0) ax[p] = a;
 }
 
 typedef double ad4_t __attribute__((ext_vector_type(4)));
@@ -2208,11 +2231,14 @@
     void prune_mark(int retry_mode, bool hinted) const {
         const bool hint = hinted && c.hint_shift;
         unsigned long long *sum = reinterpret_cast<unsigned long long *>(f.sched_ctr + SCHED_SUM) + (fm.prune ? 0 : 1);
-        hipLaunchKernelGGL(prune_mark_kernel, dim3((unsigned)f.nb), dim3(256), 0, s, xb.planes, xb.scale, c.xx, c.N, d, dpad,
+        const bool bucket = c.plane0_bucket && c.anchor_of;
+        hipLaunchKernelGGL(bucket ? prune_mark_kernel<true> : prune_mark_kernel<false>, dim3((unsigned)f.nb), dim3(256), 0, s,
+                           xb.planes, xb.scale, c.xx, c.N, d, dpad,
                            f.wt, (int)f.Mpad, f.wscale, c.ww, f.summary, (int)c.M, seeds, order, f.gap, (int)f.Mg, f.ulist,
                            (int)f.Mpad, f.ucount, f.sched_ctr, sum, fm.prune ? 0 : 1, hint ? c.hint_dist : nullptr,
                            hint ? c.hint_shift : nullptr, f.retry, retry_len(), retry_mode,
-                           (uint32_t)(c.M / 8 > 96 ? c.M / 8 : 96), fm.k2 ? f.nnub : nullptr);
+                           (uint32_t)(c.M / 8 > 96 ? c.M / 8 : 96), fm.k2 ? f.nnub : nullptr, f.wn0, c.plane0_bucket,
+                           (int)c.bucket_pitch, c.bucket_ax);
     }
 
     int gaps(hipStream_t gs) const {
@@ -2416,6 +2442,18 @@
 };
 }
 
+int dbgsom::launch_bucket_plane(const void *xplanes, int64_t N, int64_t d, const int32_t *order, int64_t pitch,
+                                int8_t *plane0_bucket, int32_t *bucket_ax, hipStream_t s) {
+    const int64_t dpad = filter_dpad(d);
+    DBGSOM_REQUIRE(xplanes && order && plane0_bucket && bucket_ax, "null pointer");
+    DBGSOM_REQUIRE(N >= 1 && N < 0x7fffffff && pitch >= dpad && pitch % 16 == 0 && pitch <= 0x7fffffff, "bad bucket plane shape");
+    PlaneBuf xb;
+    carve_planes(&xb, (char *)const_cast<void *>(xplanes), N, d);
+    hipLaunchKernelGGL(bucket_plane_kernel, dim3((unsigned)((N + 3) / 4)), dim3(256), 0, s, xb.planes, (int)dpad, order, N,
+                       (int)pitch, plane0_bucket, bucket_ax);
+    return launch_status("bucket_plane_kernel");
+}
+
 int dbgsom::launch_bmu_filtered(const FilteredCall &call) {
     FilterForm form;
     const char *rejected = form.resolve(call.seed_stride, call.sweep_planes, call.k, call.refine_rows, call.defer_dist, call.N,
@@ -2433,6 +2471,10 @@
     DBGSOM_REQUIRE(!call.anchor_of || (call.anchors && call.order && !call.prev_idx && call.n_anchors >= 1 &&
                                        call.n_anchors <= ANCHOR_MAX && form.prune && !form.seed_full && call.k == 1),
                    "anchor seeds: the stateless k = 1 pruning form, with the anchors and the bucket order");
+    DBGSOM_REQUIRE((call.plane0_bucket == nullptr) == (call.bucket_ax == nullptr) &&
+                       (!call.plane0_bucket || (call.anchor_of && call.bucket_pitch >= filter_dpad(call.d) &&
+                                                call.bucket_pitch % 64 == 0 && is_aligned(call.plane0_bucket, 128))),
+                   "the bucket plane comes with its digit norms, on an anchor-seeded call");
     DBGSOM_REQUIRE(call.anchor_of || (call.prev_idx == nullptr) == (call.order == nullptr),
                    "prev_idx and order come as a pair (both NULL = stateless two-pass search)");
     DBGSOM_REQUIRE(is_aligned(call.X, 16) && (call.ldx * (int64_t)dtype_size(call.x_dtype)) % 16 == 0 &&
@@ -2502,6 +2544,19 @@
     return DBGSOM_OK;
 }
 
+int dbgsom_bmu_filtered_lists(const void *workspace_dev, int64_t N, int64_t d, int64_t M, uint16_t *lists_host,
+                              int64_t n_groups, void *stream) {
+    DBGSOM_REQUIRE(workspace_dev && lists_host, "null pointer");
+    DBGSOM_REQUIRE(N >= 1 && d >= 1 && M >= 1 && M <= SW_MAX_M, "bad shape");
+    FilterWs f;
+    carve_filter(&f, (char *)const_cast<void *>(workspace_dev), N, d, M);
+    DBGSOM_REQUIRE(n_groups == f.nb, "n_groups must be ceil(N / 128)");
+    DBGSOM_HIP_CHECK(hipMemcpy2DAsync(lists_host, (size_t)M * 2, f.ulist, (size_t)f.Mpad * 2, (size_t)M * 2, (size_t)f.nb,
+                                      hipMemcpyDeviceToHost, (hipStream_t)stream));
+    DBGSOM_HIP_CHECK(hipStreamSynchronize((hipStream_t)stream));
+    return DBGSOM_OK;
+}
+
 int dbgsom_bmu_filtered_gaps(const void *workspace_dev, int64_t N, int64_t d, int64_t M, float *gap_host, void *stream) {
     DBGSOM_REQUIRE(workspace_dev && gap_host, "null pointer");
     DBGSOM_REQUIRE(N >= 1 && d >= 1 && M >= 1 && M <= PRUNE_MAX_M, "no gap table: M outside [1, 8192]");
diff --git a/dbgsom_amd/csrc/filter_form.h b/dbgsom_amd/csrc/filter_form.h
--- a/dbgsom_amd/csrc/filter_form.h
+++ b/dbgsom_amd/csrc/filter_form.h
@@ -16,6 +16,8 @@
     const int64_t p = (d + FKT - 1) / FKT * FKT;
     return p < 2 * FKT ? 2 * FKT : p;
 }
+
+inline int64_t bucket_plane_pitch(int64_t d) { return filter_dpad(d); }
 
 struct __attribute__((visibility("hidden"))) FilterForm {
     bool seed_full = false;
diff --git a/include/dbgsom_hip.h b/include/dbgsom_hip.h
--- a/include/dbgsom_hip.h
+++ b/include/dbgsom_hip.h
@@ -101,6 +101,8 @@
                                      uint32_t *counts_host, int64_t n_counts, void *stream);
 int dbgsom_bmu_filtered_gaps(const void *workspace_dev, int64_t N, int64_t d, int64_t M, float *gap_host,
                              void *stream);
+int dbgsom_bmu_filtered_lists(const void *workspace_dev, int64_t N, int64_t d, int64_t M, uint16_t *lists_host,
+                              int64_t n_groups, void *stream);
 int dbgsom_bmu_filtered_anchored(const void *X_dev, int x_dtype, int64_t N, int64_t d, int64_t ldx,
                                  const double *xx_dev, const void *xplanes_dev, const double *W_dev,
                                  int64_t M, const double *ww_dev, const double *anchors_dev, int n_anchors,
@@ -301,6 +303,8 @@
 int dbgsom_ctx_filter_counts(dbgsom_ctx *ctx, uint32_t *counts_host, int64_t n);
 int dbgsom_ctx_read_anchors(dbgsom_ctx *ctx, int64_t *n_anchors, double *anchors_host, int32_t *anchor_of_host,
                             int32_t *order_host, int32_t *aseed_host);
+int dbgsom_ctx_filter_lists(dbgsom_ctx *ctx, uint16_t *lists_host, int64_t n_groups);
+int dbgsom_ctx_read_bucket_plane(dbgsom_ctx *ctx, int natural, int64_t *pitch, int8_t *plane_host, int32_t *ax_host);
 int dbgsom_ctx_refine_counts(dbgsom_ctx *ctx, uint64_t *out4);
 int dbgsom_ctx_phase_ms(dbgsom_ctx *ctx, double *ms8);
 
```

After: 335.4 million samples/s/epoch. -31.7%, worse.
